# MooreThreads/LiteGS

Hardware: NVIDIA H100
Metric: forward+backward views/sec @1080p 1M Gaussians (higher is better)
Workload: dtype f32

## Files before the change

### include/litegs_b200.h

```cpp
#ifndef LITEGS_B200_H
#define LITEGS_B200_H

#include <stddef.h>
#include <stdint.h>

#ifdef __cplusplus
extern "C" {
#endif

#define LGS_ERR_ARG 10001
#define LGS_ERR_WORKSPACE 10002
#define LGS_REC_FLOATS 12
#define LGS_GRAD_FLOATS 12

const char* lgs_last_error(void);
int lgs_abi_version(void);


int lgs_frustum_culling_aabb(const float* aabb_origin, const float* aabb_ext, const float* frustumplane, int M, int V,
                             uint8_t* visibility, int* visible_num, int64_t* visible_chunk_id, void* stream);

int lgs_cull_compact_activate(int sh_degree, const int64_t* visible_chunk_id, const int* visible_chunks_num,
                              const float* view_matrix, int V, const float* position, const float* scale,
                              const float* rotation, const float* sh_base, const float* sh_rest, const float* opacity,
                              int C, int S, int A, float* act_position, float* act_scale, float* act_rotation,
                              float* color, float* act_opacity, void* stream);

int lgs_activate_backward(int sh_degree, const int64_t* visible_chunk_id, const int* visible_chunks_num,
                          const float* view_matrix, int V, const float* position, const float* scale,
                          const float* rotation, const float* opacity, int C, int S, int A, int rest_dim,
                          int true_sigmoid_grad, const float* g_act_position, const float* g_act_scale,
                          const float* g_act_rotation, const float* g_color, const float* g_act_opacity,
                          float* g_position, float* g_scale, float* g_rotation, float* g_sh_base, float* g_sh_rest,
                          float* g_opacity, void* stream);


int lgs_mvp_transform_forward(const float* world_position, const float* view_matrix, const float* proj_matrix,
                              const int* valid_length, int V, int N, float* view_position, float* ndc_position, void* stream);
int lgs_mvp_transform_backward(const float* grad_ndc_pos, const float* grad_view_pos, const float* view_matrix,
                               const float* proj_matrix, const float* view_pos, const int* valid_length, int V, int N,
                               float* grad_world_pos, void* stream);

int lgs_create_transform_matrix_forward(const float* quaternion, const float* scale, const int* valid_length, int N,
                                        float* transform, void* stream);
int lgs_create_transform_matrix_backward(const float* transform_grad, const float* quaternion, const float* scale,
                                         const int* valid_length, int N, float* grad_quaternion, float* grad_scale,
                                         void* stream);

int lgs_jacobian_rayspace(const float* view_pos, const float* proj_matrix, const int* valid_length, int V, int N,
                          int output_h, int output_w, float* jacobian, void* stream);

int lgs_create_cov2d_forward(const float* J, const float* view_matrix, const float* transform_matrix,
                             const int* valid_length, int V, int N, float* cov2d, void* stream);
int lgs_create_cov2d_backward(const float* cov2d_grad, const float* J, const float* view_matrix,
                              const float* transform_matrix, const int* valid_length, int V, int N,
                              float* transform_matrix_grad, void* stream);

int lgs_eigh_and_inv_2x2_forward(const float* input, const int* valid_length, int V, int N, float* val, float* vec,
                                 float* inv, void* stream);
int lgs_inv_2x2_backward(const float* inv_matrix, const float* grad_inv, const int* valid_length, int V, int N,
                         float* grad_matrix, void* stream);

int lgs_sh2rgb_forward(int degree, const float* sh_base, const float* sh_rest, const float* dirs, int V, int N,
                       float* rgb, void* stream);
int lgs_sh2rgb_backward(int degree, const float* rgb_grad, int sh_rest_dim, const float* dirs, int V, int N,
                        float* sh_base_grad, float* sh_rest_grad, float* dir_grad, void* stream);


int lgs_get_allocate_size(const float* ndc, const float* view_space_z, const float* inv_cov2d, const float* opacity,
                          const int* valid_length, int V, int N, int height, int width, int tile_h, int tile_w,
                          int* left_up, int* right_down, int* allocate_size, void* stream);

int lgs_create_table_workspace_bytes(int V, int cap, size_t* bytes);
int lgs_create_table(const float* ndc, const float* inv_cov2d, const float* opacity, const int* offset,
                     const int64_t* depth_sorted_pointid, int V, int N, int cap, int height, int width, int tile_h,
                     int tile_w, int* sorted_tile_id, int* sorted_point_id, void* workspace, size_t workspace_bytes,
                     void* stream);

int lgs_tile_range(const int* table_tile_id, int V, int table_length, int max_tile_id, int fix_last, int* tile_range,
                   void* stream);

int lgs_tile_range_u16(const unsigned short* table_tile_id, int V, int table_length, int max_tile_id, int fix_last,
                       int* tile_range, void* stream);

int lgs_set_sort_impl(int impl);
int lgs_set_radix_form(int onesweep);
int lgs_sort_pairs_u16_workspace_bytes(int n, size_t* bytes);
int lgs_sort_pairs_u16(const unsigned short* keys_in, unsigned short* keys_out, const unsigned* vals_in, unsigned* vals_out,
                       int n, int begin_bit, int end_bit, void* workspace, size_t workspace_bytes, void* stream);
int lgs_sort_pairs_u32_workspace_bytes(int n, size_t* bytes);
int lgs_sort_pairs_u32(const unsigned* keys_in, unsigned* keys_out, const unsigned* vals_in, unsigned* vals_out, int n,
                       int begin_bit, int end_bit, void* workspace, size_t workspace_bytes, void* stream);
int lgs_sort_pairs_u32_rebased(const unsigned* keys_in, unsigned* keys_out, const unsigned* vals_in, unsigned* vals_out, int n,
                               unsigned bias, int end_bit, void* workspace, size_t workspace_bytes, void* stream);
int lgs_scan_gathered_workspace_bytes(int n, size_t* bytes);
int lgs_scan_gathered(const int* counts, const unsigned* order, int n, int* out, void* workspace,
                      size_t workspace_bytes, void* stream);

int lgs_view_params(const int* counters , int S, int pair_capacity,
                    int planned_depth_bits, int* params ,
                    int* sticky , void* stream);
int lgs_sort_pairs_u32_dev(const unsigned* keys_in, unsigned* keys_out, const unsigned* vals_in, unsigned* vals_out, int capacity,
                           const int* n_dev, const unsigned* bias_dev, int end_bit, void* workspace, size_t workspace_bytes, void* stream);
int lgs_sort_pairs_u16_dev(const unsigned short* keys_in, unsigned short* keys_out, const unsigned* vals_in, unsigned* vals_out,
                           int capacity, const int* n_dev, int begin_bit, int end_bit, void* workspace, size_t workspace_bytes,
                           void* stream);
int lgs_sort_pairs_u32k_dev(const unsigned* keys_in, unsigned* keys_out, const unsigned* vals_in, unsigned* vals_out, int capacity,
                            const int* n_dev, int begin_bit, int end_bit, void* workspace, size_t workspace_bytes, void* stream);
int lgs_scan_gathered_dev(const int* counts, const unsigned* order, int capacity, const int* n_dev, int* out, void* workspace,
                          size_t workspace_bytes, void* stream);
int lgs_emit_pairs_dev(const float* packed_params, const int* offset, const unsigned* order, int n_capacity, const int* n_dev, int cap,
                       int img_h, int img_w, int tile_h, int tile_w, int key_bits , void* keys, int* vals,
                       int* valid_pairs , void* stream);
int lgs_tile_range_u16_dev(const unsigned short* table_tile_id, int capacity, const int* length_dev, int max_tile_id, int fix_last,
                           int* tile_range, void* stream);
int lgs_tile_range_dev(const int* table_tile_id, int capacity, const int* length_dev, int max_tile_id, int fix_last, int* tile_range,
                       void* stream);


int lgs_pack_params(const float* ndc, const float* cov2d_inv, const float* color, const float* opacity, int V, int N,
                    int img_h, int img_w, float* packed_params, void* stream);

int lgs_rasterize_forward_packed(const int* sorted_points, const int* start_index, const float* packed_params,
                                 const int* specific_tiles, int n_specific, int V, int N, int cap, int img_h, int img_w,
                                 int tile_h, int tile_w, int enable_statistic, int clamp_zero, float* img,
                                 float* transmittance, short* last_contributor, int* fragment_count,
                                 float* fragment_weight, int* tile_work, void* stream);

int lgs_tile_order(const int* work, int V, int ntile, int* order, void* stream);

int lgs_rasterize_backward(const int* sorted_points, const int* start_index, const float* packed_params,
                           const int* specific_tiles, int n_specific, const float* final_transmittance,
                           const short* last_contributor, const float* d_img, const float* d_trans_img,
                           const float* clamped_img, const float* grad_inv_scaler, int V, int N, int cap, int img_h, int img_w, int tile_h,
                           int tile_w, int enable_statistic, float* packed_grad, float* d_ndc, float* d_cov2d_inv,
                           float* d_color, float* d_opacity, float* err_sum, float* err_square_sum, void* stream);

int lgs_set_staging(int bulk);
int lgs_set_backward_reduce(int deferred);
int lgs_set_warps_per_block(int wpb);
int lgs_set_forward_pairs(int on);
int lgs_set_backward_kernel(int version);
int lgs_set_deterministic(int on);
int lgs_set_err_square_mode(int mode);


int lgs_project_forward(int sh_degree, const int64_t* visible_chunk_id, const int* visible_chunks_num,
                        const float* view_matrix, const float* proj_matrix, const float* position, const float* scale,
                        const float* rotation, const float* sh_base, const float* sh_rest, const float* opacity, int C,
                        int S, int A, int img_h, int img_w, int tile_h, int tile_w, float* packed_params,
                        unsigned* depth_key, unsigned* iota, int* tile_count, int* totals, const float* filter_3d, int antialiased,
                        void* stream);

int lgs_emit_pairs(const float* packed_params, const int* offset, const unsigned* order, int n, int cap, int img_h,
                   int img_w, int tile_h, int tile_w, int* keys, int* vals, void* stream);
int lgs_emit_pairs_u16(const float* packed_params, const int* offset, const unsigned* order, int n, int cap, int img_h,
                       int img_w, int tile_h, int tile_w, unsigned short* keys, int* vals, void* stream);

int lgs_project_backward(int sh_degree, const int64_t* visible_chunk_id, const int* visible_chunks_num,
                         const float* view_matrix, const float* proj_matrix, const float* position, const float* scale,
                         const float* rotation, const float* opacity, int C, int S, int A, int rest_dim, int img_h,
                         int img_w, int true_sigmoid_grad, const float* packed_grad, const float* grad_inv_scaler,
                         int zero_outputs, float* g_position, float* g_scale, float* g_rotation, float* g_sh_base,
                         float* g_sh_rest, float* g_opacity, float* touched, float* cam_partials, float* d_cam,
                         const float* filter_3d, int antialiased, void* stream);

int lgs_create_viewproj_forward(const float* view_params, const float* recp_tan_half_fov_x, int V, int img_h, int img_w,
                                float z_near, float z_far, float* view_matrix, float* proj_matrix, float* viewproj_matrix,
                                float* frustumplane, void* stream);
int lgs_create_viewproj_backward(const float* view_matrix_grad, const float* proj_matrix_grad, const float* viewproj_matrix_grad,
                                 const float* view_params, const float* recp_tan_half_fov_x, int V, int img_h, int img_w,
                                 float z_near, float z_far, float* grad_view_params, float* grad_recp_tan_half_fov_x, void* stream);


int lgs_adam_update_chunk(float* param, const float* grad, float* exp_avg, float* exp_avg_sq,
                          const int64_t* visible_index, const int* valid_length, int R, int C, int S, int A, double lr,
                          double b1, double b2, double eps, void* stream);
int lgs_adam_update_primitive(float* param, const float* grad, float* exp_avg, float* exp_avg_sq,
                              const int64_t* primitive_visible, int R, int N, double lr, double b1, double b2,
                              double eps, void* stream);

int lgs_mark_visible_chunks(const int64_t* visible_chunk_id, const int* visible_chunks_num, int A, float* touched, void* stream);
int lgs_adam_step_dense(float* const* params, const int* rows_per_param, const float* lr_per_param, float* grad,
                        float* exp_avg, float* exp_avg_sq, float* touched, int C, int S, double b1, double b2, double eps,
                        int clear_grad, void* stream);

int lgs_sparse_chunk_op(void* A, const void* B, const int64_t* visible_chunk_ids, const int* visible_count, int dtype,
                        int op, int ele_num, int chunks, int alloc_chunks, int chunk_size, void* stream);

int lgs_nvls_allreduce_f32(float* multicast_ptr, size_t n_floats, int rank, int world, int ctas, void* stream);


int lgs_morton_codes(const float* xyz, const float* lo3, const float* hi3, int N, int bits, long long* codes, void* stream);
int lgs_permute_rows(const float* src, const long long* idx, int R, int N, float* dst, void* stream);
int lgs_cluster_aabb(const float* xyz, const float* scale, const float* rot, int C, int S, float* origin, float* extend, void* stream);
int lgs_filter_3d(const float* position, int C, int S, const float* view, const float* proj, const int* hw, int V,
                  float* filter_3d, void* stream);


int lgs_ssim_num_block_sums(int B, int CH, int H, int W, int* count);
int lgs_ssim_forward(const float* img1, const float* img2, int B, int CH, int H, int W, float C1, float C2, int l1_mode,
                     float ssim_weight, float* map, float* dm_dmu1, float* dm_dsigma1_sq, float* dm_dsigma12,
                     float* block_sums, void* stream);
int lgs_ssim_backward(const float* img1, const float* img2, const float* dL_dmap, float uniform_chain, const float* dm_dmu1,
                      const float* dm_dsigma1_sq, const float* dm_dsigma12, int B, int CH, int H, int W, int l1_mode,
                      float ssim_weight, float* dL_dimg1, void* stream);

#ifdef __cplusplus
}
#endif
#endif
```

### litegs_b200/_lib.py

```python
from __future__ import annotations

import ctypes
import os

_HERE = os.path.dirname(os.path.abspath(__file__))
LIB_PATH = os.environ.get("LITEGS_B200_LIB") or os.path.join(_HERE, "liblitegs_b200.so")

_P, _I, _D, _Z, _F = ctypes.c_void_p, ctypes.c_int, ctypes.c_double, ctypes.c_size_t, ctypes.c_float

SIGNATURES = {
    "lgs_frustum_culling_aabb": [_P, _P, _P, _I, _I, _P, _P, _P, _P],
    "lgs_cull_compact_activate": [_I, _P, _P, _P, _I, _P, _P, _P, _P, _P, _P, _I, _I, _I, _P, _P, _P, _P, _P, _P],
    "lgs_activate_backward": [_I, _P, _P, _P, _I, _P, _P, _P, _P, _I, _I, _I, _I, _I, _P, _P, _P, _P, _P,
                              _P, _P, _P, _P, _P, _P, _P],
    "lgs_mvp_transform_forward": [_P, _P, _P, _P, _I, _I, _P, _P, _P],
    "lgs_mvp_transform_backward": [_P, _P, _P, _P, _P, _P, _I, _I, _P, _P],
    "lgs_create_transform_matrix_forward": [_P, _P, _P, _I, _P, _P],
    "lgs_create_transform_matrix_backward": [_P, _P, _P, _P, _I, _P, _P, _P],
    "lgs_jacobian_rayspace": [_P, _P, _P, _I, _I, _I, _I, _P, _P],
    "lgs_create_cov2d_forward": [_P, _P, _P, _P, _I, _I, _P, _P],
    "lgs_create_cov2d_backward": [_P, _P, _P, _P, _P, _I, _I, _P, _P],
    "lgs_eigh_and_inv_2x2_forward": [_P, _P, _I, _I, _P, _P, _P, _P],
    "lgs_inv_2x2_backward": [_P, _P, _P, _I, _I, _P, _P],
    "lgs_sh2rgb_forward": [_I, _P, _P, _P, _I, _I, _P, _P],
    "lgs_sh2rgb_backward": [_I, _P, _I, _P, _I, _I, _P, _P, _P, _P],
    "lgs_get_allocate_size": [_P, _P, _P, _P, _P, _I, _I, _I, _I, _I, _I, _P, _P, _P, _P],
    "lgs_create_table_workspace_bytes": [_I, _I, ctypes.POINTER(_Z)],
    "lgs_create_table": [_P, _P, _P, _P, _P, _I, _I, _I, _I, _I, _I, _I, _P, _P, _P, _Z, _P],
    "lgs_tile_range": [_P, _I, _I, _I, _I, _P, _P],
    "lgs_tile_range_u16": [_P, _I, _I, _I, _I, _P, _P],
    "lgs_sort_pairs_u16_workspace_bytes": [_I, ctypes.POINTER(_Z)],
    "lgs_sort_pairs_u16": [_P, _P, _P, _P, _I, _I, _I, _P, _Z, _P],
    "lgs_emit_pairs_u16": [_P, _P, _P, _I, _I, _I, _I, _I, _I, _P, _P, _P],
    "lgs_sort_pairs_u32_workspace_bytes": [_I, ctypes.POINTER(_Z)],
    "lgs_sort_pairs_u32": [_P, _P, _P, _P, _I, _I, _I, _P, _Z, _P],
    "lgs_sort_pairs_u32_rebased": [_P, _P, _P, _P, _I, ctypes.c_uint, _I, _P, _Z, _P],
    "lgs_scan_gathered_workspace_bytes": [_I, ctypes.POINTER(_Z)],
    "lgs_scan_gathered": [_P, _P, _I, _P, _P, _Z, _P],
    "lgs_view_params": [_P, _I, _I, _I, _P, _P, _P],
    "lgs_sort_pairs_u32_dev": [_P, _P, _P, _P, _I, _P, _P, _I, _P, _Z, _P],
    "lgs_sort_pairs_u16_dev": [_P, _P, _P, _P, _I, _P, _I, _I, _P, _Z, _P],
    "lgs_sort_pairs_u32k_dev": [_P, _P, _P, _P, _I, _P, _I, _I, _P, _Z, _P],
    "lgs_scan_gathered_dev": [_P, _P, _I, _P, _P, _P, _Z, _P],
    "lgs_emit_pairs_dev": [_P, _P, _P, _I, _P, _I, _I, _I, _I, _I, _I, _P, _P, _P, _P],
    "lgs_tile_range_u16_dev": [_P, _I, _P, _I, _I, _P, _P],
    "lgs_tile_range_dev": [_P, _I, _P, _I, _I, _P, _P],
    "lgs_pack_params": [_P, _P, _P, _P, _I, _I, _I, _I, _P, _P],
    "lgs_rasterize_forward_packed": [_P, _P, _P, _P, _I, _I, _I, _I, _I, _I, _I, _I, _I, _I, _P, _P, _P, _P, _P, _P, _P],
    "lgs_tile_order": [_P, _I, _I, _P, _P],
    "lgs_rasterize_backward": [_P, _P, _P, _P, _I, _P, _P, _P, _P, _P, _P, _I, _I, _I, _I, _I, _I, _I, _I,
                               _P, _P, _P, _P, _P, _P, _P, _P],
    "lgs_set_staging": [_I],
    "lgs_set_sort_impl": [_I],
    "lgs_set_radix_form": [_I],
    "lgs_set_warps_per_block": [_I],
    "lgs_set_backward_reduce": [_I],
    "lgs_set_backward_kernel": [_I],
    "lgs_set_forward_pairs": [_I],
    "lgs_set_err_square_mode": [_I],
    "lgs_set_deterministic": [_I],
    "lgs_project_forward": [_I, _P, _P, _P, _P, _P, _P, _P, _P, _P, _P, _I, _I, _I, _I, _I, _I, _I, _P, _P, _P, _P, _P, _P, _I, _P],
    "lgs_emit_pairs": [_P, _P, _P, _I, _I, _I, _I, _I, _I, _P, _P, _P],
    "lgs_project_backward": [_I, _P, _P, _P, _P, _P, _P, _P, _P, _I, _I, _I, _I, _I, _I, _I, _P, _P, _I,
                             _P, _P, _P, _P, _P, _P, _P, _P, _P, _P, _I, _P],
    "lgs_create_viewproj_forward": [_P, _P, _I, _I, _I, _F, _F, _P, _P, _P, _P, _P],
    "lgs_create_viewproj_backward": [_P, _P, _P, _P, _P, _I, _I, _I, _F, _F, _P, _P, _P],
    "lgs_adam_update_chunk": [_P, _P, _P, _P, _P, _P, _I, _I, _I, _I, _D, _D, _D, _D, _P],
    "lgs_adam_update_primitive": [_P, _P, _P, _P, _P, _I, _I, _D, _D, _D, _D, _P],
    "lgs_sparse_chunk_op": [_P, _P, _P, _P, _I, _I, _I, _I, _I, _I, _P],
    "lgs_mark_visible_chunks": [_P, _P, _I, _P, _P],
    "lgs_nvls_allreduce_f32": [_P, _Z, _I, _I, _I, _P],
    "lgs_morton_codes": [_P, _P, _P, _I, _I, _P, _P],
    "lgs_permute_rows": [_P, _P, _I, _I, _P, _P],
    "lgs_cluster_aabb": [_P, _P, _P, _I, _I, _P, _P, _P],
    "lgs_filter_3d": [_P, _I, _I, _P, _P, _P, _I, _P, _P],
    "lgs_adam_step_dense": [_P, _P, _P, _P, _P, _P, _P, _I, _I, _D, _D, _D, _I, _P],
    "lgs_ssim_num_block_sums": [_I, _I, _I, _I, ctypes.POINTER(_I)],
    "lgs_ssim_forward": [_P, _P, _I, _I, _I, _I, _F, _F, _I, _F, _P, _P, _P, _P, _P, _P],
    "lgs_ssim_backward": [_P, _P, _P, _F, _P, _P, _P, _I, _I, _I, _I, _I, _F, _P, _P],
}
NO_STATUS = {"lgs_last_error": ctypes.c_char_p, "lgs_abi_version": ctypes.c_int}

_lib = None


class LiteGSB200Error(RuntimeError):
    pass


def load() -> ctypes.CDLL:
    global _lib
    if _lib is not None:
        return _lib
    if not os.path.exists(LIB_PATH):
        raise LiteGSB200Error(
            f"{LIB_PATH} not found: build it with `python -m litegs_b200.build` (nvcc, sm_90a). "
            "litegs_b200 has no CPU or PyTorch fallback.")
    lib = ctypes.CDLL(LIB_PATH)
    for name, argtypes in SIGNATURES.items():
        fn = getattr(lib, name)
        fn.argtypes = argtypes
        fn.restype = ctypes.c_int
    for name, restype in NO_STATUS.items():
        fn = getattr(lib, name)
        fn.argtypes = []
        fn.restype = restype
    _lib = lib
    return lib


def exported_symbols():
    return list(SIGNATURES) + list(NO_STATUS)


def call(name: str, *args) -> None:
    lib = load()
    rc = getattr(lib, name)(*args)
    if rc != 0:
        msg = lib.lgs_last_error()
        raise LiteGSB200Error(f"{name} failed (code {rc}): {msg.decode() if msg else ''}")
```

### litegs_b200/csrc/raster.cu

```cuda
#include "common.cuh"

#define FULL_MASK 0xffffffffu
#define LOG2E 1.4426950408889634f
#define ALPHA_MIN (1.0f / 256.0f)
#define ALPHA_MAX (255.0f / 256.0f)
#define T_MIN (1.0f / 8192.0f)
#define WARPS_PER_BLOCK 4

__device__ __forceinline__ float fast_ex2(float x)
{
    float y;
    asm("ex2.approx.ftz.f32 %0, %1;" : "=f"(y) : "f"(x));
    return y;
}
__device__ __forceinline__ float fast_rcp(float x)
{
    float y;
    asm("rcp.approx.ftz.f32 %0, %1;" : "=f"(y) : "f"(x));
    return y;
}

__device__ __forceinline__ float2 add2(float2 a, float2 b) { return make_float2(__fadd_rn(a.x, b.x), __fadd_rn(a.y, b.y)); }
__device__ __forceinline__ float2 mul2(float2 a, float2 b) { return make_float2(__fmul_rn(a.x, b.x), __fmul_rn(a.y, b.y)); }
__device__ __forceinline__ float2 fma2(float2 a, float2 b, float2 c) { return make_float2(__fmaf_rn(a.x, b.x, c.x), __fmaf_rn(a.y, b.y, c.y)); }

__device__ __forceinline__ void blend_pixel(float a, float cr, float cg, float cb, float& Ts, float& Cr, float& Cg, float& Cb,
                                            float& nf, float ts_min, float a_min, float neg_ki)
{
    asm("{\n"
        ".reg .pred pa, pk;\n"
        ".reg .f32 w;\n"
        "setp.gt.f32 pa, %0, %9;\n"
        "@pa add.f32 %4, %4, 0f3F800000;\n"
        "setp.ge.and.f32 pk, %5, %10, pa;\n"
        "mul.f32 w, %5, %0;\n"
        "@pk fma.rn.f32 %1, %6, w, %1;\n"
        "@pk fma.rn.f32 %2, %7, w, %2;\n"
        "@pk fma.rn.f32 %3, %8, w, %3;\n"
        "@pk fma.rn.f32 %0, %11, w, %0;\n"
        "}\n"
        : "+f"(Ts), "+f"(Cr), "+f"(Cg), "+f"(Cb), "+f"(nf)
        : "f"(a), "f"(cr), "f"(cg), "f"(cb), "f"(ts_min), "f"(a_min), "f"(neg_ki));
}

__device__ __forceinline__ unsigned smem_u32(const void* p) { return (unsigned)__cvta_generic_to_shared(p); }
__device__ __forceinline__ void cp_async16(void* dst, const void* src)
{
    asm volatile("cp.async.cg.shared.global [%0], [%1], 16;\n" ::"r"(smem_u32(dst)), "l"(src));
}
__device__ __forceinline__ void cp_async_commit() { asm volatile("cp.async.commit_group;\n" ::); }
template <int N> __device__ __forceinline__ void cp_async_wait() { asm volatile("cp.async.wait_group %0;\n" ::"n"(N)); }

__device__ __forceinline__ void mbar_init(uint64_t* bar, unsigned count)
{
    asm volatile("mbarrier.init.shared::cta.b64 [%0], %1;\n" ::"r"(smem_u32(bar)), "r"(count));
}
__device__ __forceinline__ void mbar_expect_tx(uint64_t* bar, unsigned bytes)
{
    asm volatile("mbarrier.arrive.expect_tx.shared::cta.b64 _, [%0], %1;\n" ::"r"(smem_u32(bar)), "r"(bytes));
}
__device__ __forceinline__ bool mbar_try_wait(uint64_t* bar, unsigned parity)
{
    unsigned ok;
    asm volatile(
        "{\n"
        ".reg .pred p;\n"
        "mbarrier.try_wait.parity.shared::cta.b64 p, [%1], %2;\n"
        "selp.u32 %0, 1, 0, p;\n"
        "}\n"
        : "=r"(ok)
        : "r"(smem_u32(bar)), "r"(parity)
        : "memory");
    return ok != 0;
}
__device__ __forceinline__ void mbar_wait(uint64_t* bar, unsigned parity)
{
    while (!mbar_try_wait(bar, parity)) {}
}
__device__ __forceinline__ void bulk_g2s(void* dst, const void* src, unsigned bytes, uint64_t* bar)
{
    asm volatile("cp.async.bulk.shared::cluster.global.mbarrier::complete_tx::bytes [%0], [%1], %2, [%3];\n" ::"r"(smem_u32(dst)),
                 "l"(src), "r"(bytes), "r"(smem_u32(bar))
                 : "memory");
}

template <bool BULK>
struct Stager {
    SplatRec* buf;
    uint64_t* bar;
    unsigned phase_bits;
    unsigned pending;
    int lane;
    __device__ __forceinline__ void init(SplatRec* b, uint64_t* m, int ln)
    {
        buf = b; bar = m; lane = ln; phase_bits = 0; pending = 0;
        if (BULK) {
            if (lane == 0) { mbar_init(&bar[0], 1); mbar_init(&bar[1], 1); }
            asm volatile("fence.mbarrier_init.release.cluster;\n" ::);
            __syncwarp();
        }
    }
    __device__ __forceinline__ void issue(int which, const SplatRec* __restrict__ recs, int id)
    {
        SplatRec* dst = buf + which * 32 + lane;
        if (BULK) {
            unsigned live = __ballot_sync(FULL_MASK, id >= 0);
            if (lane == 0) mbar_expect_tx(&bar[which], (unsigned)__popc(live) * (unsigned)sizeof(SplatRec));
            __syncwarp();
            if (id >= 0) bulk_g2s(dst, recs + id, (unsigned)sizeof(SplatRec), &bar[which]);
            pending |= (1u << which);
        } else {
            if (id >= 0) {
                const char* src = (const char*)(recs + id);
                cp_async16((char*)dst, src);
                cp_async16((char*)dst + 16, src + 16);
                cp_async16((char*)dst + 32, src + 32);
            }
            cp_async_commit();
        }
    }
    template <bool PRE = false>
    __device__ __forceinline__ void wait(int which, bool more_in_flight)
    {
        if (BULK) {
            mbar_wait(&bar[which], (phase_bits >> which) & 1u);
            phase_bits ^= (1u << which);
            pending &= ~(1u << which);
            if (PRE) { prescale(which); __syncwarp(); }
        } else {
            if (more_in_flight) cp_async_wait<1>(); else cp_async_wait<0>();
            if (PRE) prescale(which);
            __syncwarp();
        }
    }
    __device__ __forceinline__ void prescale(int which)
    {
        SplatRec* r = buf + which * 32 + lane;
        const float2 ab = *reinterpret_cast<const float2*>(&r->A);
        const float2 co = *reinterpret_cast<const float2*>(&r->C);
        *reinterpret_cast<float2*>(&r->A) = make_float2((-0.5f * LOG2E) * ab.x, (-LOG2E) * ab.y);
        r->C = (-0.5f * LOG2E) * co.x;
        r->depth = co.y * (256.0f / 255.0f);
    }
    __device__ __forceinline__ void drain()
    {
        if (BULK) {
            if (pending & 1u) wait(0, false);
            if (pending & 2u) wait(1, false);
        } else {
            cp_async_wait<0>();
        }
    }
};

__global__ void pack_kernel(const float* __restrict__ ndc, const float* __restrict__ inv_cov, const float* __restrict__ color,
                            const float* __restrict__ opac, SplatRec* __restrict__ recs, int N, int H, int W)
{
    int i = blockIdx.x * blockDim.x + threadIdx.x, b = blockIdx.y;
    if (i >= N) return;
    size_t o4 = (size_t)b * 4 * N + i, o3 = (size_t)b * 3 * N + i;
    SplatRec r;
    r.px = __fsub_rn(__fmul_rn(__fmul_rn(__fadd_rn(ndc[o4], 1.0f), 0.5f), (float)W), 0.5f);
    r.py = __fsub_rn(__fmul_rn(__fmul_rn(__fadd_rn(ndc[o4 + N], 1.0f), 0.5f), (float)H), 0.5f);
    r.depth = ndc[o4 + 2 * (size_t)N];
    r.A = inv_cov[o4]; r.B = inv_cov[o4 + N]; r.C = inv_cov[o4 + 3 * (size_t)N];
    r.o = opac[i];
    r.r = color[o3]; r.g = color[o3 + N]; r.b = color[o3 + 2 * (size_t)N];
    r.pad0 = 0.f; r.pad1 = 0.f;
    recs[(size_t)b * N + i] = r;
}

template <int TH, int TW, bool STAT, bool BULK, bool PAIRS = false>
__global__ void __launch_bounds__(32 * WARPS_PER_BLOCK) raster_forward_kernel(
    const int* __restrict__ sorted, const int* __restrict__ start_index, const SplatRec* __restrict__ recs,
    const int* __restrict__ tiles, int n_sel, float* __restrict__ img, float* __restrict__ Tout, unsigned short* __restrict__ last,
    int* __restrict__ frag_count, float* __restrict__ frag_weight, int* __restrict__ tile_work, int gx, int ntile, int cap, int N,
    int Hp, int Wp, int clamp_zero)
{
    constexpr int PPT = TH * TW / 32;
    __shared__ __align__(128) SplatRec s_rec[WARPS_PER_BLOCK][2][32];
    __shared__ __align__(8) uint64_t s_bar[WARPS_PER_BLOCK][2];
    const int lane = threadIdx.x, warp = threadIdx.y, b = blockIdx.y;
    const int slot = blockIdx.x * blockDim.y + warp;
    int tile_id;
    if (tiles != nullptr) tile_id = (slot < n_sel) ? tiles[(size_t)b * n_sel + slot] : 0;
    else tile_id = slot + 1;
    if (tile_id <= 0 || tile_id > ntile) return;

    const int* rg = start_index + (size_t)b * (ntile + 2);
    const int start = rg[tile_id];
    int count = (start < 0) ? 0 : (rg[tile_id + 1] - start);
    if (count < 0) count = 0;
    recs += (size_t)b * N;
    const int* ids = sorted + (size_t)b * cap + (start < 0 ? 0 : start);

    const int x = ((tile_id - 1) % gx) * TW + lane % TW;
    const int y0 = ((tile_id - 1) / gx) * TH + (lane / TW) * PPT;
    const float fx = (float)x, fy0 = (float)y0;

    constexpr float KS = 256.0f / 255.0f, KI = 255.0f / 256.0f;
    constexpr float TS_MIN = T_MIN * KI, A_MIN_S = ALPHA_MIN * KS;
    float Ts[PPT], Cr[PPT], Cg[PPT], Cb[PPT], nf[PPT];
#pragma unroll
    for (int j = 0; j < PPT; j++) { Ts[j] = KI; Cr[j] = Cg[j] = Cb[j] = 0.0f; nf[j] = 0.0f; }

    if (count > 0) {
        Stager<BULK> st;
        st.init(&s_rec[warp][0][0], &s_bar[warp][0], lane);
        const int nchunks = (count + 31) >> 5;
        int id_cur = (lane < count) ? ids[lane] : -1;
        st.issue(0, recs, id_cur);
        int id_next = (32 + lane < count) ? ids[32 + lane] : -1;
        bool done = false;
        for (int c = 0; c < nchunks && !done; c++) {
            const bool more = (c + 1 < nchunks);
            if (more) {
                st.issue((c + 1) & 1, recs, id_next);
                int nn = (c + 2) * 32 + lane;
                id_next = (nn < count) ? ids[nn] : -1;
            }
            st.template wait<true>(c & 1, more);
            const SplatRec* chunk = &s_rec[warp][c & 1][0];
            const int nk = min(32, count - c * 32);
            int my_id = 0;
            if (STAT) my_id = ids[c * 32 + min(lane, nk - 1)];
            for (int k = 0; k < nk; k++) {
                if ((k & 3) == 0) {
                    float tmax = Ts[0];
#pragma unroll
                    for (int j = 1; j < PPT; j++) tmax = fmaxf(tmax, Ts[j]);
                    if (!__any_sync(FULL_MASK, tmax > TS_MIN)) { done = true; break; }
                }
                const float4 q0 = *reinterpret_cast<const float4*>(&chunk[k].px);
                const float4 q1 = *reinterpret_cast<const float4*>(&chunk[k].C);
                const float2 q2 = *reinterpret_cast<const float2*>(&chunk[k].b);
                const float cb = q2.x;
                const float dx = q0.x - fx, dy0 = q0.y - fy0;
                const float a2 = q0.z, b2 = q0.w, c2 = q1.x;
                const float base = a2 * dx * dx, lin = b2 * dx;
                const float os = q2.y;
                int fcount = 0; float wsum = 0.f;
                if (PAIRS && !STAT) {
                    const float2 dy02 = make_float2(dy0, dy0), c22 = make_float2(c2, c2), lin2 = make_float2(lin, lin),
                                 base2 = make_float2(base, base), os2 = make_float2(os, os);
                    const float2 cr2 = make_float2(q1.z, q1.z), cg2 = make_float2(q1.w, q1.w), cb2 = make_float2(cb, cb),
                                 nki2 = make_float2(-KI, -KI);
#pragma unroll
                    for (int p = 0; p < PPT / 2; p++) {
                        const float2 dy = add2(dy02, make_float2(-(float)(2 * p), -(float)(2 * p + 1)));
                        const float2 pw = fma2(dy, fma2(c22, dy, lin2), base2);
                        const float2 t = mul2(os2, make_float2(fast_ex2(pw.x), fast_ex2(pw.y)));
                        const float a0 = __saturatef(t.x), a1 = __saturatef(t.y);
                        const bool act0 = Ts[2 * p] > TS_MIN, act1 = Ts[2 * p + 1] > TS_MIN;
                        if (act0) nf[2 * p] += 1.0f;
                        if (act1) nf[2 * p + 1] += 1.0f;
                        const float2 aw = make_float2((act0 && a0 >= A_MIN_S) ? a0 : 0.0f, (act1 && a1 >= A_MIN_S) ? a1 : 0.0f);
                        const float2 w = mul2(aw, make_float2(Ts[2 * p], Ts[2 * p + 1]));
                        const float2 r2 = fma2(cr2, w, make_float2(Cr[2 * p], Cr[2 * p + 1]));
                        const float2 g2 = fma2(cg2, w, make_float2(Cg[2 * p], Cg[2 * p + 1]));
                        const float2 b2_ = fma2(cb2, w, make_float2(Cb[2 * p], Cb[2 * p + 1]));
                        const float2 tn = fma2(nki2, w, make_float2(Ts[2 * p], Ts[2 * p + 1]));
                        Cr[2 * p] = r2.x; Cr[2 * p + 1] = r2.y; Cg[2 * p] = g2.x; Cg[2 * p + 1] = g2.y;
                        Cb[2 * p] = b2_.x; Cb[2 * p + 1] = b2_.y; Ts[2 * p] = tn.x; Ts[2 * p + 1] = tn.y;
                    }
                } else {
#pragma unroll
                for (int j = 0; j < PPT; j++) {
                    const float dy = dy0 - (float)j;
                    const float pw = fmaf(dy, fmaf(c2, dy, lin), base);
                    const float a = __saturatef(os * fast_ex2(pw));
                    if (STAT) {
                        const bool ok = (Ts[j] > TS_MIN) && (a >= A_MIN_S);
                        if (ok) { fcount++; wsum += a * Ts[j]; }
                    }
                    blend_pixel(a, q1.z, q1.w, cb, Ts[j], Cr[j], Cg[j], Cb[j], nf[j], TS_MIN, A_MIN_S, -KI);
                }
                }
                if (STAT) {
                    fcount = __reduce_add_sync(FULL_MASK, fcount);
#pragma unroll
                    for (int o = 16; o > 0; o >>= 1) wsum += __shfl_xor_sync(FULL_MASK, wsum, o);
                    int pid = __shfl_sync(FULL_MASK, my_id, k);
                    if (lane == 0 && fcount > 0) {
                        atomicAdd(&frag_count[(size_t)b * N + pid], fcount);
                        atomicAdd(&frag_weight[(size_t)b * N + pid], wsum);
                    }
                }
            }
            __syncwarp();
        }
        st.drain();
    }

    const size_t plane = (size_t)Hp * Wp;
#pragma unroll
    for (int j = 0; j < PPT; j++) {
        const size_t po = (size_t)(y0 + j) * Wp + x;
        const float lo = clamp_zero ? 0.0f : -3.4028234663852886e38f;
        img[((size_t)b * 3 + 0) * plane + po] = fmaxf(fminf(Cr[j], 1.0f), lo);
        img[((size_t)b * 3 + 1) * plane + po] = fmaxf(fminf(Cg[j], 1.0f), lo);
        img[((size_t)b * 3 + 2) * plane + po] = fmaxf(fminf(Cb[j], 1.0f), lo);
        Tout[(size_t)b * plane + po] = Ts[j] * KS;
        last[(size_t)b * plane + po] = (unsigned short)__float2uint_rn(fminf(nf[j], 65535.0f));
    }
    if (tile_work != nullptr) {
        float m = nf[0];
#pragma unroll
        for (int j = 1; j < PPT; j++) m = fmaxf(m, nf[j]);
        const int mi = __reduce_max_sync(FULL_MASK, (int)fminf(m, 65535.0f));
        if (lane == 0) tile_work[(size_t)b * ntile + tile_id - 1] = mi;
    }
}

__device__ __forceinline__ float butterfly8(const float (&v)[8], int lane)
{
    const bool h16 = lane & 16, h8 = lane & 8, h4 = lane & 4;
    float u[4], w[2];
#pragma unroll
    for (int i = 0; i < 4; i++) {
        float send = h16 ? v[i] : v[i + 4], keep = h16 ? v[i + 4] : v[i];
        u[i] = keep + __shfl_xor_sync(FULL_MASK, send, 16);
    }
#pragma unroll
    for (int i = 0; i < 2; i++) {
        float send = h8 ? u[i] : u[i + 2], keep = h8 ? u[i + 2] : u[i];
        w[i] = keep + __shfl_xor_sync(FULL_MASK, send, 8);
    }
    float send = h4 ? w[0] : w[1], keep = h4 ? w[1] : w[0];
    float z = keep + __shfl_xor_sync(FULL_MASK, send, 4);
    z += __shfl_xor_sync(FULL_MASK, z, 2);
    z += __shfl_xor_sync(FULL_MASK, z, 1);
    return z;
}

#define LGS_RG 3
#define LGS_ROWF 36
template <int TH, int TW, bool STAT, bool TRANS, bool BULK, bool DEFER>
__global__ void __launch_bounds__(32 * WARPS_PER_BLOCK) raster_backward_kernel(
    const int* __restrict__ sorted, const int* __restrict__ start_index, const SplatRec* __restrict__ recs,
    const int* __restrict__ tiles, int n_sel, const float* __restrict__ Tfinal, const unsigned short* __restrict__ last,
    const float* __restrict__ d_img, const float* __restrict__ d_trans, const float* __restrict__ clamped_img,
    float* __restrict__ grad, int gx, int ntile, int cap, int N, int Hp, int Wp)
{
    constexpr int PPT = TH * TW / 32;
    constexpr int NV = STAT ? 10 : 9;
    constexpr float KS = 256.0f / 255.0f, A_MIN_S = ALPHA_MIN * KS;
    __shared__ __align__(128) SplatRec s_rec[WARPS_PER_BLOCK][2][32];
    __shared__ __align__(8) uint64_t s_bar[WARPS_PER_BLOCK][2];
    __shared__ __align__(16) float s_acc[DEFER ? WARPS_PER_BLOCK : 1][DEFER ? LGS_RG * NV : 1][LGS_ROWF];
    const int lane = threadIdx.x, warp = threadIdx.y, b = blockIdx.y;
    const int slot = blockIdx.x * blockDim.y + warp;
    int tile_id;
    if (tiles != nullptr) tile_id = (slot < n_sel) ? tiles[(size_t)b * n_sel + slot] : 0;
    else tile_id = slot + 1;
    if (tile_id <= 0 || tile_id > ntile) return;
    const int* rg = start_index + (size_t)b * (ntile + 2);
    const int start = rg[tile_id];
    if (start < 0) return;
    recs += (size_t)b * N;
    grad += (size_t)b * N * LGS_GRAD_FLOATS;
    const int* ids = sorted + (size_t)b * cap + start;

    const int x = ((tile_id - 1) % gx) * TW + lane % TW;
    const int y0 = ((tile_id - 1) / gx) * TH + (lane / TW) * PPT;
    const float fx = (float)x, fy0 = (float)y0;
    const size_t plane = (size_t)Hp * Wp;

    float T[PPT], g0[PPT], g1[PPT], g2[PPT], S[PPT], gt[PPT];
    int nl[PPT];
    int kmax = 0;
#pragma unroll
    for (int j = 0; j < PPT; j++) {
        const size_t po = (size_t)(y0 + j) * Wp + x;
        T[j] = Tfinal[(size_t)b * plane + po];
        g0[j] = d_img[((size_t)b * 3 + 0) * plane + po];
        g1[j] = d_img[((size_t)b * 3 + 1) * plane + po];
        g2[j] = d_img[((size_t)b * 3 + 2) * plane + po];
        if (clamped_img != nullptr) {
            if (!(clamped_img[((size_t)b * 3 + 0) * plane + po] > 0.0f)) g0[j] = 0.0f;
            if (!(clamped_img[((size_t)b * 3 + 1) * plane + po] > 0.0f)) g1[j] = 0.0f;
            if (!(clamped_img[((size_t)b * 3 + 2) * plane + po] > 0.0f)) g2[j] = 0.0f;
        }
        gt[j] = TRANS ? d_trans[(size_t)b * plane + po] * T[j] : 0.0f;
        S[j] = 0.0f;
        nl[j] = (int)last[(size_t)b * plane + po];
        kmax = max(kmax, nl[j]);
    }
    kmax = __reduce_max_sync(FULL_MASK, kmax);
    if (kmax <= 0) return;

    int pend = 0, pid0 = 0, pid1 = 0, pid2 = 0;
    auto flush = [&]() {
        __syncwarp();
        if (lane < pend * NV) {
            const float4* r4 = reinterpret_cast<const float4*>(&s_acc[DEFER ? warp : 0][DEFER ? lane : 0][0]);
            float4 x0 = r4[0], x1 = r4[1], x2 = r4[2], x3 = r4[3], x4 = r4[4], x5 = r4[5], x6 = r4[6], x7 = r4[7];
            float sum = (((x0.x + x0.y) + (x0.z + x0.w)) + ((x1.x + x1.y) + (x1.z + x1.w))) +
                        (((x2.x + x2.y) + (x2.z + x2.w)) + ((x3.x + x3.y) + (x3.z + x3.w))) +
                        ((((x4.x + x4.y) + (x4.z + x4.w)) + ((x5.x + x5.y) + (x5.z + x5.w))) +
                         (((x6.x + x6.y) + (x6.z + x6.w)) + ((x7.x + x7.y) + (x7.z + x7.w))));
            const int sp = lane / NV, v = lane - sp * NV;
            const int pid = sp == 0 ? pid0 : (sp == 1 ? pid1 : pid2);
            atomicAdd(&grad[(size_t)pid * LGS_GRAD_FLOATS + v], sum);
        }
        __syncwarp();
        pend = 0;
    };
    Stager<BULK> st;
    st.init(&s_rec[warp][0][0], &s_bar[warp][0], lane);
    const int nchunks = (kmax + 31) >> 5;
    int c0 = nchunks - 1;
    int id_cur = (c0 * 32 + lane < kmax) ? ids[c0 * 32 + lane] : -1;
    st.issue(0, recs, id_cur);
    int id_next = (c0 >= 1) ? ids[(c0 - 1) * 32 + lane] : -1;
    for (int v = 0; v < nchunks; v++) {
        const int c = nchunks - 1 - v;
        const bool more = (c >= 1);
        const int id_this = id_cur;
        if (more) {
            st.issue((v + 1) & 1, recs, id_next);
            id_cur = id_next;
            id_next = (c >= 2) ? ids[(c - 2) * 32 + lane] : -1;
        }
        st.wait(v & 1, more);
        const SplatRec* chunk = &s_rec[warp][v & 1][0];
        const int nk = min(32, kmax - c * 32);
        for (int kk = nk - 1; kk >= 0; kk--) {
            const int k = c * 32 + kk;
            const float4 q0 = *reinterpret_cast<const float4*>(&chunk[kk].px);
            const float4 q1 = *reinterpret_cast<const float4*>(&chunk[kk].C);
            const float cb = chunk[kk].b;
            const float dx = q0.x - fx, dy0 = q0.y - fy0;
            const float a2 = (-0.5f * LOG2E) * q0.z, b2 = (-LOG2E) * q0.w, c2 = (-0.5f * LOG2E) * q1.x;
            const float base = a2 * dx * dx, lin = b2 * dx;
            const float os = q1.y * KS;
            float s0 = 0.f, s1 = 0.f, s2 = 0.f, dr = 0.f, dg = 0.f, db = 0.f, esq = 0.f;
            bool any = false;
#pragma unroll
            for (int j = 0; j < PPT; j++) {
                const float dy = dy0 - (float)j;
                const float pw = fmaf(dy, fmaf(c2, dy, lin), base);
                const float G = fast_ex2(pw);
                const float at = q1.y * G;
                if (k < nl[j] && os * G >= A_MIN_S) {
                    any = true;
                    const float a = fminf(at, ALPHA_MAX);
                    const float rc = fast_rcp(1.0f - a);
                    const float Tj = fminf(1.0f, T[j] * rc);
                    T[j] = Tj;
                    const float w = a * Tj;
                    dr = fmaf(w, g0[j], dr); dg = fmaf(w, g1[j], dg); db = fmaf(w, g2[j], db);
                    const float diff = fmaf(q1.z, g0[j], fmaf(q1.w, g1[j], cb * g2[j])) - S[j];
                    float da = Tj * diff;
                    if (TRANS) da -= gt[j] * rc;
                    S[j] = fmaf(a, diff, S[j]);
                    if (STAT) { const float go = G * da; esq = fmaf(go, go, esq); }
                    const float dpw = at * da;
                    s0 += dpw; s1 = fmaf(dpw, dy, s1); s2 = fmaf(dpw * dy, dy, s2);
                }
            }
            if (__any_sync(FULL_MASK, any)) {
                float v8[8];
                const float u0 = dx * s0;
                v8[0] = u0;
                v8[1] = s1;
                v8[2] = dx * u0;
                v8[3] = dx * s1;
                v8[4] = s2;
                v8[5] = dr; v8[6] = dg; v8[7] = db;
                float dop = s0;
                const int pid = __shfl_sync(FULL_MASK, id_this, kk);
                if (DEFER) {
                    float* row = &s_acc[DEFER ? warp : 0][DEFER ? pend * NV : 0][lane];
#pragma unroll
                    for (int v = 0; v < 8; v++) row[v * LGS_ROWF] = v8[v];
                    row[8 * LGS_ROWF] = dop;
                    if (STAT) row[9 * LGS_ROWF] = esq;
                    if (pend == 0) pid0 = pid; else if (pend == 1) pid1 = pid; else pid2 = pid;
                    pend++;
                    if (pend == LGS_RG) flush();
                } else {
                    const float tot = butterfly8(v8, lane);
#pragma unroll
                    for (int o = 16; o > 0; o >>= 1) dop += __shfl_xor_sync(FULL_MASK, dop, o);
                    if (STAT) {
#pragma unroll
                        for (int o = 16; o > 0; o >>= 1) esq += __shfl_xor_sync(FULL_MASK, esq, o);
                    }
                    int slotv = -1; float val = 0.f;
                    if ((lane & 3) == 0) { slotv = ((lane >> 4) & 1) * 4 + ((lane >> 3) & 1) * 2 + ((lane >> 2) & 1); val = tot; }
                    else if (lane == 1) { slotv = 8; val = dop; }
                    else if (STAT && lane == 2) { slotv = 9; val = esq; }
                    if (slotv >= 0) atomicAdd(&grad[(size_t)pid * LGS_GRAD_FLOATS + slotv], val);
                }
            }
        }
        __syncwarp();
    }
    if (DEFER && pend > 0) flush();
    st.drain();
}

__device__ __forceinline__ float2 bc2(float a) { return make_float2(a, a); }

#define LGS_DET_SCALE 68719476736.0
template <int TH, int TW, bool STAT, bool TRANS, bool DET = false>
__global__ void __launch_bounds__(32 * WARPS_PER_BLOCK) raster_backward_v2_kernel(
    const int* __restrict__ sorted, const int* __restrict__ start_index, const SplatRec* __restrict__ recs,
    const int* __restrict__ tiles, int n_sel, const float* __restrict__ Tfinal, const unsigned short* __restrict__ last,
    const float* __restrict__ d_img, const float* __restrict__ d_trans, const float* __restrict__ clamped_img,
    float* __restrict__ grad, int gx, int ntile, int cap, int N, int Hp, int Wp, int err_mode)
{
    constexpr int PPT = TH * TW / 32, NP = PPT / 2;
    static_assert(PPT % 2 == 0, "pixels per lane must pair up");
    constexpr int NV = STAT ? 10 : 9;
    constexpr float KS = 256.0f / 255.0f, A_MIN_S = ALPHA_MIN * KS;
    __shared__ __align__(128) SplatRec s_rec[WARPS_PER_BLOCK][2][32];
    __shared__ __align__(8) uint64_t s_bar[WARPS_PER_BLOCK][2];
    __shared__ __align__(16) float s_acc[WARPS_PER_BLOCK][LGS_RG * NV][LGS_ROWF];
    __shared__ int s_pid[WARPS_PER_BLOCK][4];
    const int lane = threadIdx.x, warp = threadIdx.y, b = blockIdx.y;
    const int slot = blockIdx.x * blockDim.y + warp;
    int tile_id;
    if (tiles != nullptr) tile_id = (slot < n_sel) ? tiles[(size_t)b * n_sel + slot] : 0;
    else tile_id = slot + 1;
    if (tile_id <= 0 || tile_id > ntile) return;
    const int* rg = start_index + (size_t)b * (ntile + 2);
    const int start = rg[tile_id];
    if (start < 0) return;
    recs += (size_t)b * N;
    grad += (size_t)b * N * LGS_GRAD_FLOATS * (DET ? 2 : 1);
    const int* ids = sorted + (size_t)b * cap + start;

    const int x = ((tile_id - 1) % gx) * TW + lane % TW;
    const int y0 = ((tile_id - 1) / gx) * TH + (lane / TW) * PPT;
    const float fx = (float)x, fy0 = (float)y0;
    const size_t plane = (size_t)Hp * Wp;

    float2 T[NP], g0[NP], g1[NP], g2[NP], S[NP], ngt[NP];
    int nl[PPT];
    int kmax = 0;
#pragma unroll
    for (int j = 0; j < PPT; j++) {
        const size_t po = (size_t)(y0 + j) * Wp + x;
        float t = Tfinal[(size_t)b * plane + po];
        float a0 = d_img[((size_t)b * 3 + 0) * plane + po];
        float a1 = d_img[((size_t)b * 3 + 1) * plane + po];
        float a2 = d_img[((size_t)b * 3 + 2) * plane + po];
        if (clamped_img != nullptr) {
            if (!(clamped_img[((size_t)b * 3 + 0) * plane + po] > 0.0f)) a0 = 0.0f;
            if (!(clamped_img[((size_t)b * 3 + 1) * plane + po] > 0.0f)) a1 = 0.0f;
            if (!(clamped_img[((size_t)b * 3 + 2) * plane + po] > 0.0f)) a2 = 0.0f;
        }
        const float gtj = TRANS ? -(d_trans[(size_t)b * plane + po] * t) : 0.0f;
        if (j & 1) { T[j / 2].y = t; g0[j / 2].y = a0; g1[j / 2].y = a1; g2[j / 2].y = a2; ngt[j / 2].y = gtj; S[j / 2].y = 0.f; }
        else       { T[j / 2].x = t; g0[j / 2].x = a0; g1[j / 2].x = a1; g2[j / 2].x = a2; ngt[j / 2].x = gtj; S[j / 2].x = 0.f; }
        nl[j] = (int)last[(size_t)b * plane + po];
        kmax = max(kmax, nl[j]);
    }
    kmax = __reduce_max_sync(FULL_MASK, kmax);
    if (kmax <= 0) return;

    int pend = 0;
    auto flush = [&]() {
        __syncwarp();
        if (lane < pend * NV) {
            const float4* r4 = reinterpret_cast<const float4*>(&s_acc[warp][lane][0]);
            const float4 x0 = r4[0], x1 = r4[1], x2 = r4[2], x3 = r4[3], x4 = r4[4], x5 = r4[5], x6 = r4[6], x7 = r4[7];
            float2 p0 = add2(make_float2(x0.x, x0.y), make_float2(x0.z, x0.w));
            float2 p1 = add2(make_float2(x1.x, x1.y), make_float2(x1.z, x1.w));
            float2 p2 = add2(make_float2(x2.x, x2.y), make_float2(x2.z, x2.w));
            float2 p3 = add2(make_float2(x3.x, x3.y), make_float2(x3.z, x3.w));
            float2 p4 = add2(make_float2(x4.x, x4.y), make_float2(x4.z, x4.w));
            float2 p5 = add2(make_float2(x5.x, x5.y), make_float2(x5.z, x5.w));
            float2 p6 = add2(make_float2(x6.x, x6.y), make_float2(x6.z, x6.w));
            float2 p7 = add2(make_float2(x7.x, x7.y), make_float2(x7.z, x7.w));
            p0 = add2(p0, p1); p2 = add2(p2, p3); p4 = add2(p4, p5); p6 = add2(p6, p7);
            p0 = add2(p0, p2); p4 = add2(p4, p6);
            p0 = add2(p0, p4);
            const float sum = p0.x + p0.y;
            const int sp = lane / NV, v = lane - sp * NV;
            const int pid = s_pid[warp][sp];
            if (DET) {
                unsigned long long* gq = reinterpret_cast<unsigned long long*>(grad);
                atomicAdd(&gq[(size_t)pid * LGS_GRAD_FLOATS + v], (unsigned long long)__double2ll_rn((double)sum * LGS_DET_SCALE));
            } else {
                atomicAdd(&grad[(size_t)pid * LGS_GRAD_FLOATS + v], sum);
            }
        }
        __syncwarp();
        pend = 0;
    };
    Stager<false> st;
    st.init(&s_rec[warp][0][0], &s_bar[warp][0], lane);
    const int nchunks = (kmax + 31) >> 5;
    int c0 = nchunks - 1;
    int id_cur = (c0 * 32 + lane < kmax) ? ids[c0 * 32 + lane] : -1;
    st.issue(0, recs, id_cur);
    int id_next = (c0 >= 1) ? ids[(c0 - 1) * 32 + lane] : -1;
    for (int v = 0; v < nchunks; v++) {
        const int c = nchunks - 1 - v;
        const bool more = (c >= 1);
        const int id_this = id_cur;
        if (more) {
            st.issue((v + 1) & 1, recs, id_next);
            id_cur = id_next;
            id_next = (c >= 2) ? ids[(c - 2) * 32 + lane] : -1;
        }
        st.template wait<true>(v & 1, more);
        const SplatRec* chunk = &s_rec[warp][v & 1][0];
        const int nk = min(32, kmax - c * 32);
        for (int kk = nk - 1; kk >= 0; kk--) {
            const int k = c * 32 + kk;
            const float4 q0 = *reinterpret_cast<const float4*>(&chunk[kk].px);
            const float4 q1 = *reinterpret_cast<const float4*>(&chunk[kk].C);
            const float2 q2 = *reinterpret_cast<const float2*>(&chunk[kk].b);
            const float cb = q2.x;
            const float dx = q0.x - fx, dy0 = q0.y - fy0;
            const float a2 = q0.z, b2 = q0.w, c2 = q1.x;
            const float base = a2 * dx * dx, lin = b2 * dx;
            const float2 os2 = bc2(q2.y), o2 = bc2(q1.y), c22 = bc2(c2), lin2 = bc2(lin), base2 = bc2(base);
            const float2 cr2 = bc2(q1.z), cg2 = bc2(q1.w), cb2 = bc2(cb), dy02 = bc2(dy0);
            float2 s0, s1, s2, dr, dg, db;
            float esq = 0.f, runx = 0.f, runy = 0.f;
            bool any = false;
#pragma unroll
            for (int p = 0; p < NP; p++) {
                const float2 dy = add2(dy02, make_float2(-(float)(2 * p), -(float)(2 * p + 1)));
                const float2 pw = fma2(dy, fma2(c22, dy, lin2), base2);
                float2 G = make_float2(fast_ex2(pw.x), fast_ex2(pw.y));
                const float2 tt = mul2(os2, G);
                const bool ok0 = (tt.x >= A_MIN_S) && (k < nl[2 * p]);
                const bool ok1 = (tt.y >= A_MIN_S) && (k < nl[2 * p + 1]);
                any |= ok0 | ok1;
                G.x = ok0 ? G.x : 0.0f;
                G.y = ok1 ? G.y : 0.0f;
                const float2 at = mul2(o2, G);
                const float2 a = make_float2(fminf(at.x, ALPHA_MAX), fminf(at.y, ALPHA_MAX));
                const float2 om = fma2(a, bc2(-1.0f), bc2(1.0f));
                const float2 rc = make_float2(fast_rcp(om.x), fast_rcp(om.y));
                const float2 Tn = mul2(T[p], rc);
                T[p] = Tn;
                const float2 w = mul2(a, Tn);
                const float2 cgd = fma2(cr2, g0[p], fma2(cg2, g1[p], mul2(cb2, g2[p])));
                const float2 diff = fma2(S[p], bc2(-1.0f), cgd);
                float2 da = mul2(Tn, diff);
                if (TRANS) da = fma2(ngt[p], rc, da);
                S[p] = fma2(a, diff, S[p]);
                const float2 dpw = mul2(at, da);
                const float2 td = mul2(dpw, dy);
                if (p == 0) {
                    dr = mul2(w, g0[p]); dg = mul2(w, g1[p]); db = mul2(w, g2[p]);
                    s0 = dpw; s1 = td; s2 = mul2(td, dy);
                } else {
                    dr = fma2(w, g0[p], dr); dg = fma2(w, g1[p], dg); db = fma2(w, g2[p], db);
                    s0 = add2(s0, dpw);
                    s1 = add2(s1, td);
                    s2 = fma2(td, dy, s2);
                }
                if (STAT) {
                    const float2 go = mul2(G, da);
                    if (err_mode == 1) {
                        if (__any_sync(FULL_MASK, ok0 | ok1)) {
                            runx += go.x; runy += go.y;
                            esq = fmaf(runx, runx, fmaf(runy, runy, esq));
                        }
                    } else {
                        esq = fmaf(go.x, go.x, fmaf(go.y, go.y, esq));
                    }
                }
            }
            if (__any_sync(FULL_MASK, any)) {
                const float m0 = s0.x + s0.y, m1 = s1.x + s1.y, m2 = s2.x + s2.y;
                const float u0 = dx * m0;
                if (lane == kk) s_pid[warp][pend] = id_this;
                float* row = &s_acc[warp][pend * NV][lane];
                row[0 * LGS_ROWF] = u0;
                row[1 * LGS_ROWF] = m1;
                row[2 * LGS_ROWF] = dx * u0;
                row[3 * LGS_ROWF] = dx * m1;
                row[4 * LGS_ROWF] = m2;
                row[5 * LGS_ROWF] = dr.x + dr.y;
                row[6 * LGS_ROWF] = dg.x + dg.y;
                row[7 * LGS_ROWF] = db.x + db.y;
                row[8 * LGS_ROWF] = m0;
                if (STAT) row[9 * LGS_ROWF] = esq;
                pend++;
                if (pend == LGS_RG) flush();
            }
        }
        __syncwarp();
    }
    if (pend > 0) flush();
    st.drain();
}

__global__ void det_to_float_kernel(const long long* __restrict__ q, float* __restrict__ g, size_t n)
{
    size_t i = (size_t)blockIdx.x * blockDim.x + threadIdx.x;
    if (i < n) g[i] = (float)((double)q[i] * (1.0 / LGS_DET_SCALE));
}

__global__ void unpack_kernel(const float* __restrict__ grad, const SplatRec* __restrict__ recs, const float* __restrict__ inv_scaler,
                              int N, int H, int W, float* __restrict__ d_ndc, float* __restrict__ d_cov, float* __restrict__ d_color,
                              float* __restrict__ d_opac, float* __restrict__ err_sum, float* __restrict__ err_sq)
{
    int i = blockIdx.x * blockDim.x + threadIdx.x, b = blockIdx.y;
    if (i >= N) return;
    const float s = inv_scaler ? inv_scaler[0] : 1.0f;
    const float4* g4 = reinterpret_cast<const float4*>(grad + ((size_t)b * N + i) * LGS_GRAD_FLOATS);
    const float4 a = g4[0], c = g4[1], e = g4[2];
    const SplatRec r = recs[(size_t)b * N + i];
    LgsRasterGrad g;
    lgs_finish_raster_grad(a, c, e, r.A, r.B, r.C, r.o, g);
    size_t o4 = (size_t)b * 4 * N + i, o3 = (size_t)b * 3 * N + i;
    d_ndc[o4] = g.dmx * 0.5f * W * s; d_ndc[o4 + N] = g.dmy * 0.5f * H * s;
    d_ndc[o4 + 2 * (size_t)N] = 0.f; d_ndc[o4 + 3 * (size_t)N] = 0.f;
    d_cov[o4] = g.dA * s; d_cov[o4 + N] = g.dB * 0.5f * s; d_cov[o4 + 2 * (size_t)N] = g.dB * 0.5f * s; d_cov[o4 + 3 * (size_t)N] = g.dC * s;
    d_color[o3] = c.y * s; d_color[o3 + N] = c.z * s; d_color[o3 + 2 * (size_t)N] = c.w * s;
    if (b == 0) d_opac[i] = g.dop * s;
    if (err_sum) err_sum[(size_t)b * N + i] = 0.f;
    if (err_sq) err_sq[(size_t)b * N + i] = e.y;
}

__global__ void __launch_bounds__(1024) tile_order_kernel(const int* __restrict__ work, int ntile, int* __restrict__ order)
{
    __shared__ int s_cnt[1024];
    __shared__ int s_warp[32];
    const int t = threadIdx.x, b = blockIdx.x;
    const int* w = work + (size_t)b * ntile;
    s_cnt[t] = 0;
    __syncthreads();
    for (int i = t; i < ntile; i += 1024) atomicAdd(&s_cnt[1023 - min(max(w[i], 0) >> 2, 1023)], 1);
    __syncthreads();
    const int c = s_cnt[t];
    int incl = c;
#pragma unroll
    for (int o = 1; o < 32; o <<= 1) { int v = __shfl_up_sync(FULL_MASK, incl, o); if ((t & 31) >= o) incl += v; }
    if ((t & 31) == 31) s_warp[t >> 5] = incl;
    __syncthreads();
    if (t < 32) {
        int v = s_warp[t], in2 = v;
#pragma unroll
        for (int o = 1; o < 32; o <<= 1) { int u = __shfl_up_sync(FULL_MASK, in2, o); if (t >= o) in2 += u; }
        s_warp[t] = in2 - v;
    }
    __syncthreads();
    s_cnt[t] = incl - c + s_warp[t >> 5];
    __syncthreads();
    for (int i = t; i < ntile; i += 1024) {
        const int pos = atomicAdd(&s_cnt[1023 - min(max(w[i], 0) >> 2, 1023)], 1);
        order[(size_t)b * ntile + pos] = i + 1;
    }
}

extern "C" int lgs_tile_order(const int* work, int V, int ntile, int* order, void* stream)
{
    LGS_REQUIRE(V >= 1 && ntile >= 1, "tile_order: bad sizes V=%d tiles=%d", V, ntile);
    tile_order_kernel<<<V, 1024, 0, (cudaStream_t)stream>>>(work, ntile, order);
    LGS_CHECK_LAUNCH("tile_order_kernel");
    return LGS_OK;
}

static int g_use_bulk = -1;
static bool use_bulk()
{
    if (g_use_bulk < 0) {
        const char* e = getenv("LGS_STAGING");
        g_use_bulk = (e && e[0] == 'b') ? 1 : 0;
    }
    return g_use_bulk == 1;
}
extern "C" int lgs_set_staging(int bulk) { g_use_bulk = bulk ? 1 : 0; return LGS_OK; }

static int g_defer = -1;
static bool use_deferred_reduce()
{
    if (g_defer < 0) {
        const char* e = getenv("LGS_BWD_REDUCE");
        g_defer = (e && e[0] == 'b') ? 0 : 1;
    }
    return g_defer == 1;
}
extern "C" int lgs_set_backward_reduce(int deferred) { g_defer = deferred ? 1 : 0; return LGS_OK; }

static int g_fwd_pairs = -1;
static bool forward_pairs()
{
    if (g_fwd_pairs < 0) {
        const char* e = getenv("LGS_FWD_PAIRS");
        g_fwd_pairs = (e && e[0] == '1') ? 1 : 0;
    }
    return g_fwd_pairs == 1;
}
extern "C" int lgs_set_forward_pairs(int on) { g_fwd_pairs = on ? 1 : 0; return LGS_OK; }

static int g_bwd = -1;
static int backward_version()
{
    if (g_bwd < 0) {
        const char* e = getenv("LGS_BWD");
        g_bwd = (e && (e[0] == '1' || (e[0] == 'v' && e[1] == '1'))) ? 1 : 2;
    }
    return g_bwd;
}
extern "C" int lgs_set_backward_kernel(int version)
{
    LGS_REQUIRE(version == 1 || version == 2, "set_backward_kernel: %d not in {1,2}", version);
    g_bwd = version;
    return LGS_OK;
}

static int g_err_mode = 1;
extern "C" int lgs_set_err_square_mode(int mode)
{
    LGS_REQUIRE(mode == 0 || mode == 1, "set_err_square_mode: %d not in {0,1}", mode);
    g_err_mode = mode;
    return LGS_OK;
}

static int g_det = -1;
static bool deterministic()
{
    if (g_det < 0) {
        const char* e = getenv("LGS_DETERMINISTIC");
        g_det = (e && e[0] == '1') ? 1 : 0;
    }
    return g_det == 1;
}
extern "C" int lgs_set_deterministic(int on) { g_det = on ? 1 : 0; return LGS_OK; }

static int g_wpb = -1;
static int warps_per_block()
{
    if (g_wpb < 0) {
        const char* e = getenv("LGS_WPB");
        int v = e ? atoi(e) : 4;
        g_wpb = (v == 1 || v == 2 || v == 4) ? v : 4;
    }
    return g_wpb;
}
extern "C" int lgs_set_warps_per_block(int wpb)
{
    LGS_REQUIRE(wpb == 1 || wpb == 2 || wpb == 4, "set_warps_per_block: %d not in {1,2,4}", wpb);
    g_wpb = wpb;
    return LGS_OK;
}

extern "C" int lgs_pack_params(const float* ndc, const float* cov2d_inv, const float* color, const float* opacity, int V, int N,
                               int img_h, int img_w, float* packed_params, void* stream)
{
    if (N == 0) return LGS_OK;
    pack_kernel<<<dim3(lgs_cdiv(N, 256), V), 256, 0, (cudaStream_t)stream>>>(ndc, cov2d_inv, color, opacity, (SplatRec*)packed_params, N,
                                                                           img_h, img_w);
    LGS_CHECK_LAUNCH("pack_kernel");
    return LGS_OK;
}

extern "C" int lgs_rasterize_forward_packed(const int* sorted_points, const int* start_index, const float* packed_params,
                                            const int* specific_tiles, int n_specific, int V, int N, int cap, int img_h, int img_w,
                                            int tile_h, int tile_w, int enable_statistic, int clamp_zero, float* img,
                                            float* transmittance, short* last_contributor, int* fragment_count,
                                            float* fragment_weight, int* tile_work, void* stream)
{
    LGS_REQUIRE(lgs_tile_ok(tile_h, tile_w), "rasterize_forward: tile %dx%d not one of 8x16, 12x16, 16x16, 8x8", tile_h, tile_w);
    LGS_REQUIRE(V >= 1 && img_h > 0 && img_w > 0, "rasterize_forward: bad sizes V=%d H=%d W=%d", V, img_h, img_w);
    int gx = (img_w + tile_w - 1) / tile_w, gy = (img_h + tile_h - 1) / tile_h;
    int ntile = gx * gy, Hp = gy * tile_h, Wp = gx * tile_w;
    int nrender = specific_tiles ? n_specific : ntile;
    if (nrender == 0) return LGS_OK;
    const int wpb = warps_per_block();
    dim3 grid(lgs_cdiv(nrender, wpb), V), block(32, wpb);
    cudaStream_t st = (cudaStream_t)stream;
    const SplatRec* recs = (const SplatRec*)packed_params;
    const bool bulk = use_bulk();
#define FWD(S, B) raster_forward_kernel<TH, TW, S, B><<<grid, block, 0, st>>>(sorted_points, start_index, recs, specific_tiles, n_specific, \
        img, transmittance, (unsigned short*)last_contributor, fragment_count, fragment_weight, tile_work, gx, ntile, cap, N, Hp, Wp, clamp_zero)
#define FWDP() raster_forward_kernel<TH, TW, false, false, true><<<grid, block, 0, st>>>(sorted_points, start_index, recs, specific_tiles, \
        n_specific, img, transmittance, (unsigned short*)last_contributor, fragment_count, fragment_weight, tile_work, gx, ntile, cap, N, Hp, Wp, clamp_zero)
    LGS_DISPATCH_TILE(tile_h, tile_w,
        if (enable_statistic) { if (bulk) FWD(true, true); else FWD(true, false); }
        else { if (bulk) FWD(false, true); else if (forward_pairs()) FWDP(); else FWD(false, false); })
#undef FWD
#undef FWDP
    LGS_CHECK_LAUNCH("raster_forward_kernel");
    return LGS_OK;
}

extern "C" int lgs_rasterize_backward(const int* sorted_points, const int* start_index, const float* packed_params,
                                      const int* specific_tiles, int n_specific, const float* final_transmittance,
                                      const short* last_contributor, const float* d_img, const float* d_trans_img,
                                      const float* clamped_img, const float* grad_inv_scaler, int V, int N, int cap, int img_h,
                                      int img_w, int tile_h,
                                      int tile_w, int enable_statistic, float* packed_grad, float* d_ndc, float* d_cov2d_inv,
                                      float* d_color, float* d_opacity, float* err_sum, float* err_square_sum, void* stream)
{
    LGS_REQUIRE(lgs_tile_ok(tile_h, tile_w), "rasterize_backward: tile %dx%d not one of 8x16, 12x16, 16x16, 8x8", tile_h, tile_w);
    LGS_REQUIRE(V >= 1 && img_h > 0 && img_w > 0, "rasterize_backward: bad sizes V=%d H=%d W=%d", V, img_h, img_w);
    int gx = (img_w + tile_w - 1) / tile_w, gy = (img_h + tile_h - 1) / tile_h;
    int ntile = gx * gy, Hp = gy * tile_h, Wp = gx * tile_w;
    int nrender = specific_tiles ? n_specific : ntile;
    cudaStream_t st = (cudaStream_t)stream;
    if (N == 0) return LGS_OK;
    LGS_CUDA(cudaMemsetAsync(packed_grad, 0, sizeof(float) * (size_t)V * N * LGS_GRAD_FLOATS, st));
    if (nrender > 0) {
        const int wpb = warps_per_block();
        dim3 grid(lgs_cdiv(nrender, wpb), V), block(32, wpb);
        const SplatRec* recs = (const SplatRec*)packed_params;
        const bool bulk = use_bulk();
        const bool trans = d_trans_img != nullptr;
        const bool defer = use_deferred_reduce() && !bulk;
        const unsigned short* lastu = (const unsigned short*)last_contributor;
        if (deterministic()) {
            const size_t nq = (size_t)V * N * LGS_GRAD_FLOATS;
            long long* q = nullptr;
            LGS_CUDA(cudaMallocAsync((void**)&q, nq * sizeof(long long), st));
            LGS_CUDA(cudaMemsetAsync(q, 0, nq * sizeof(long long), st));
#define BWD_DET(S, T) raster_backward_v2_kernel<TH, TW, S, T, true><<<grid, block, 0, st>>>(sorted_points, start_index, recs, specific_tiles, \
        n_specific, final_transmittance, lastu, d_img, d_trans_img, clamped_img, (float*)q, gx, ntile, cap, N, Hp, Wp, g_err_mode)
            LGS_DISPATCH_TILE(tile_h, tile_w,
                if (enable_statistic) { if (trans) BWD_DET(true, true); else BWD_DET(true, false); }
                else { if (trans) BWD_DET(false, true); else BWD_DET(false, false); })
#undef BWD_DET
            LGS_CHECK_LAUNCH("raster_backward_v2_kernel<DET>");
            det_to_float_kernel<<<lgs_cdiv((long long)nq, 256), 256, 0, st>>>(q, packed_grad, nq);
            LGS_CHECK_LAUNCH("det_to_float_kernel");
            LGS_CUDA(cudaFreeAsync(q, st));
        } else if (backward_version() == 2 && !bulk) {
#define BW2(S, T) raster_backward_v2_kernel<TH, TW, S, T><<<grid, block, 0, st>>>(sorted_points, start_index, recs, specific_tiles, n_specific, \
        final_transmittance, lastu, d_img, d_trans_img, clamped_img, packed_grad, gx, ntile, cap, N, Hp, Wp, g_err_mode)
            LGS_DISPATCH_TILE(tile_h, tile_w,
                if (enable_statistic) { if (trans) BW2(true, true); else BW2(true, false); }
                else { if (trans) BW2(false, true); else BW2(false, false); })
#undef BW2
            LGS_CHECK_LAUNCH("raster_backward_v2_kernel");
        } else {
#define BWD(S, T, B) if (defer) BWD2(S, T, false, true); else BWD2(S, T, B, false)
#define BWD2(S, T, B, D) raster_backward_kernel<TH, TW, S, T, B, D><<<grid, block, 0, st>>>(sorted_points, start_index, recs, specific_tiles, \
        n_specific, final_transmittance, lastu, d_img, d_trans_img, clamped_img, packed_grad, gx, ntile, cap, N, Hp, Wp)
        LGS_DISPATCH_TILE(tile_h, tile_w,
            if (enable_statistic) { if (trans) { if (bulk) BWD(true, true, true); else BWD(true, true, false); }
                                    else { if (bulk) BWD(true, false, true); else BWD(true, false, false); } }
            else { if (trans) { if (bulk) BWD(false, true, true); else BWD(false, true, false); }
                   else { if (bulk) BWD(false, false, true); else BWD(false, false, false); } })
#undef BWD
#undef BWD2
        LGS_CHECK_LAUNCH("raster_backward_kernel");
        }
    }
    if (d_ndc != nullptr) {
        unpack_kernel<<<dim3(lgs_cdiv(N, 256), V), 256, 0, st>>>(packed_grad, (const SplatRec*)packed_params, grad_inv_scaler, N, img_h, img_w,
                                                                d_ndc, d_cov2d_inv, d_color, d_opacity, err_sum, err_square_sum);
        LGS_CHECK_LAUNCH("unpack_kernel");
    }
    return LGS_OK;
}
```

### litegs_b200/fused.py

```python
from __future__ import annotations

import ctypes
import math
import os
from typing import Optional

import torch

from . import _lib

_F32, _I32, _I64 = torch.float32, torch.int32, torch.int64

CONFIG = {
    "fix_last_tile": True,
    "true_sigmoid_grad": False,
    "tile_order": os.environ.get("LGS_TILE_ORDER", "1") != "0",
}


def _ptr(t: Optional[torch.Tensor]):
    return None if t is None else t.data_ptr()


def _stream(dev):
    return torch.cuda.current_stream(dev).cuda_stream


class _OnDevice:
    __slots__ = ("ctx",)

    def __init__(self, dev):
        self.ctx = None if torch.cuda.current_device() == (dev.index if dev.index is not None else torch.cuda.current_device()) \
            else torch.cuda.device(dev)

    def __enter__(self):
        if self.ctx is not None:
            self.ctx.__enter__()

    def __exit__(self, *a):
        if self.ctx is not None:
            return self.ctx.__exit__(*a)
        return False


_on = _OnDevice


def _f32c(t: torch.Tensor, name: str) -> torch.Tensor:
    if not t.is_cuda:
        raise RuntimeError(f"{name} must be a CUDA tensor (litegs_b200 has no CPU path)")
    if t.dtype != _F32:
        raise RuntimeError(f"{name}: expected float32, got {t.dtype}")
    return t if t.is_contiguous() else t.contiguous()


def _asc(t: torch.Tensor, dtype, name: str) -> torch.Tensor:
    if not t.is_cuda:
        raise RuntimeError(f"{name} must be a CUDA tensor")
    if t.dtype != dtype:
        raise RuntimeError(f"{name}: expected {dtype}, got {t.dtype}")
    return t if t.is_contiguous() else t.contiguous()


def _vl(valid_length: Optional[torch.Tensor]):
    if valid_length is None:
        return None
    return _asc(valid_length, _I32, "valid_length")


def _tiles(img_h, img_w, th, tw):
    gy = (int(img_h) + th - 1) // th
    gx = (int(img_w) + tw - 1) // tw
    return gx, gy



def frustum_culling_aabb(aabb_origin, aabb_ext, frustumplane, feedback_buffer_arg=None, data_idx_arg=None):
    o = _f32c(aabb_origin, "aabb_origin"); e = _f32c(aabb_ext, "aabb_ext"); f = _f32c(frustumplane, "frustumplane")
    M, V = o.shape[1], f.shape[0]
    dev = o.device
    with torch.cuda.device(dev):
        vis = torch.empty(M, dtype=torch.bool, device=dev)
        num = torch.zeros(1, dtype=_I32, device=dev)
        ids = torch.arange(M, dtype=_I64, device=dev)
        _lib.call("lgs_frustum_culling_aabb", _ptr(o), _ptr(e), _ptr(f), M, V, _ptr(vis), _ptr(num), _ptr(ids), _stream(dev))
        pred = 0
        if feedback_buffer_arg is not None and data_idx_arg is not None:
            for i in range(data_idx_arg.shape[0]):
                idx = int(data_idx_arg[i])
                pred = max(pred, int(feedback_buffer_arg[idx]))
                feedback_buffer_arg[idx:idx + 1].copy_(num, non_blocking=True)
        pred = int(1.2 * pred)
        if pred <= 0:
            pred = int(num.item())
        pred = min(pred, M)
    return [vis, num, ids[:pred]]


def cull_compact_activate(sh_degree, visible_chunk_id, visible_chunks_num, view_matrix,
                          position, scale, rotation, sh_base, sh_rest, opacity):
    ids = _asc(visible_chunk_id, _I64, "visible_chunk_id"); num = _asc(visible_chunks_num, _I32, "visible_chunks_num")
    view = _f32c(view_matrix, "view_matrix")
    pos = _f32c(position, "position"); sc = _f32c(scale, "scale"); rot = _f32c(rotation, "rotation")
    s0 = _f32c(sh_base, "sh_base"); sr = _f32c(sh_rest, "sh_rest"); op = _f32c(opacity, "opacity")
    K = (int(sh_degree) + 1) ** 2
    if sr.shape[0] < K - 1:
        raise RuntimeError(f"sh_rest has {sr.shape[0]} rows, sh_degree {sh_degree} needs {K - 1}")
    C, S = pos.shape[-2:]
    A, V = ids.shape[0], view.shape[0]
    dev = pos.device
    with torch.cuda.device(dev):
        apos = torch.empty((4, A, S), dtype=_F32, device=dev)
        asc = torch.empty((3, A, S), dtype=_F32, device=dev)
        arot = torch.empty((4, A, S), dtype=_F32, device=dev)
        color = torch.empty((V, 3, A, S), dtype=_F32, device=dev)
        aop = torch.empty((1, A, S), dtype=_F32, device=dev)
        _lib.call("lgs_cull_compact_activate", int(sh_degree), _ptr(ids), _ptr(num), _ptr(view), V, _ptr(pos), _ptr(sc),
                  _ptr(rot), _ptr(s0), _ptr(sr), _ptr(op), C, S, A, _ptr(apos), _ptr(asc), _ptr(arot), _ptr(color),
                  _ptr(aop), _stream(dev))
    return [apos, asc, arot, color, aop]


def activate_backward(sh_degree, visible_chunk_id, visible_chunks_num, view_matrix,
                      position, scale, rotation, sh_base, sh_rest, opacity,
                      activated_position_grad, activated_scale_grad, activated_rotation_grad, color_grad,
                      activated_opacity_grad):
    ids = _asc(visible_chunk_id, _I64, "visible_chunk_id"); num = _asc(visible_chunks_num, _I32, "visible_chunks_num")
    view = _f32c(view_matrix, "view_matrix")
    pos = _f32c(position, "position"); sc = _f32c(scale, "scale"); rot = _f32c(rotation, "rotation")
    op = _f32c(opacity, "opacity")
    gp = _f32c(activated_position_grad, "activated_position_grad"); gs = _f32c(activated_scale_grad, "activated_scale_grad")
    gr = _f32c(activated_rotation_grad, "activated_rotation_grad"); gc = _f32c(color_grad, "color_grad")
    go = _f32c(activated_opacity_grad, "activated_opacity_grad")
    C, S = pos.shape[-2:]
    A, V, R = ids.shape[0], view.shape[0], sh_rest.shape[0]
    dev = pos.device
    with torch.cuda.device(dev):
        o_pos = torch.empty((3, A, S), dtype=_F32, device=dev)
        o_sc = torch.empty((3, A, S), dtype=_F32, device=dev)
        o_rot = torch.empty((4, A, S), dtype=_F32, device=dev)
        o_s0 = torch.empty((1, 3, A, S), dtype=_F32, device=dev)
        o_sr = torch.empty((R, 3, A, S), dtype=_F32, device=dev)
        o_op = torch.empty((1, A, S), dtype=_F32, device=dev)
        _lib.call("lgs_activate_backward", int(sh_degree), _ptr(ids), _ptr(num), _ptr(view), V, _ptr(pos), _ptr(sc), _ptr(rot),
                  _ptr(op), C, S, A, R, int(CONFIG["true_sigmoid_grad"]), _ptr(gp), _ptr(gs), _ptr(gr), _ptr(gc), _ptr(go),
                  _ptr(o_pos), _ptr(o_sc), _ptr(o_rot), _ptr(o_s0), _ptr(o_sr), _ptr(o_op), _stream(dev))
    return [o_pos, o_sc, o_rot, o_s0, o_sr, o_op]



def mvp_transform_forward(world_position, view_matrix, proj_matrix, valid_length=None):
    p = _f32c(world_position, "world_position"); vm = _f32c(view_matrix, "view_matrix"); pm = _f32c(proj_matrix, "proj_matrix")
    V, N = vm.shape[0], p.shape[1]
    dev = p.device
    with torch.cuda.device(dev):
        vp = torch.empty((V, 4, N), dtype=_F32, device=dev)
        ndc = torch.empty((V, 4, N), dtype=_F32, device=dev)
        _lib.call("lgs_mvp_transform_forward", _ptr(p), _ptr(vm), _ptr(pm), _ptr(_vl(valid_length)), V, N, _ptr(vp), _ptr(ndc), _stream(dev))
    return [vp, ndc]


def mvp_transform_backward(grad_ndc_pos, grad_view_pos, view_matrix, proj_matrix, view_pos, valid_length=None):
    gn = _f32c(grad_ndc_pos, "grad_ndc_pos"); gv = _f32c(grad_view_pos, "grad_view_pos")
    vm = _f32c(view_matrix, "view_matrix"); pm = _f32c(proj_matrix, "proj_matrix"); vp = _f32c(view_pos, "view_pos")
    V, N = gn.shape[0], gn.shape[2]
    dev = gn.device
    with torch.cuda.device(dev):
        out = torch.empty((4, N), dtype=_F32, device=dev)
        _lib.call("lgs_mvp_transform_backward", _ptr(gn), _ptr(gv), _ptr(vm), _ptr(pm), _ptr(vp), _ptr(_vl(valid_length)), V, N,
                  _ptr(out), _stream(dev))
    return out


def createTransformMatrix_forward(quaternion, scale, valid_length=None):
    q = _f32c(quaternion, "quaternion"); s = _f32c(scale, "scale")
    N = q.shape[1]
    dev = q.device
    with torch.cuda.device(dev):
        T = torch.empty((3, 3, N), dtype=_F32, device=dev)
        _lib.call("lgs_create_transform_matrix_forward", _ptr(q), _ptr(s), _ptr(_vl(valid_length)), N, _ptr(T), _stream(dev))
    return T


def createTransformMatrix_backward(transform_matrix_grad, quaternion, scale, valid_length=None):
    g = _f32c(transform_matrix_grad, "transform_matrix_grad"); q = _f32c(quaternion, "quaternion"); s = _f32c(scale, "scale")
    N = q.shape[1]
    dev = q.device
    with torch.cuda.device(dev):
        gq = torch.empty((4, N), dtype=_F32, device=dev)
        gs = torch.empty((3, N), dtype=_F32, device=dev)
        _lib.call("lgs_create_transform_matrix_backward", _ptr(g), _ptr(q), _ptr(s), _ptr(_vl(valid_length)), N, _ptr(gq), _ptr(gs),
                  _stream(dev))
    return [gq, gs]


def jacobianRayspace(translated_position, proj_matrix, output_h, output_w, valid_length=None):
    vp = _f32c(translated_position, "translated_position"); pm = _f32c(proj_matrix, "proj_matrix")
    V, N = vp.shape[0], vp.shape[2]
    dev = vp.device
    with torch.cuda.device(dev):
        J = torch.empty((V, 3, 3, N), dtype=_F32, device=dev)
        _lib.call("lgs_jacobian_rayspace", _ptr(vp), _ptr(pm), _ptr(_vl(valid_length)), V, N, int(output_h), int(output_w), _ptr(J),
                  _stream(dev))
    return J


def createCov2dDirectly_forward(J, view_matrix, transform_matrix, valid_length=None):
    j = _f32c(J, "J"); vm = _f32c(view_matrix, "view_matrix"); T = _f32c(transform_matrix, "transform_matrix")
    V, N = vm.shape[0], T.shape[2]
    dev = T.device
    with torch.cuda.device(dev):
        cov = torch.empty((V, 2, 2, N), dtype=_F32, device=dev)
        _lib.call("lgs_create_cov2d_forward", _ptr(j), _ptr(vm), _ptr(T), _ptr(_vl(valid_length)), V, N, _ptr(cov), _stream(dev))
    return cov


def createCov2dDirectly_backward(cov2d_grad, J, view_matrix, transform_matrix, valid_length=None):
    g = _f32c(cov2d_grad, "cov2d_grad"); j = _f32c(J, "J"); vm = _f32c(view_matrix, "view_matrix")
    T = _f32c(transform_matrix, "transform_matrix")
    V, N = vm.shape[0], T.shape[2]
    dev = T.device
    with torch.cuda.device(dev):
        gT = torch.empty((3, 3, N), dtype=_F32, device=dev)
        _lib.call("lgs_create_cov2d_backward", _ptr(g), _ptr(j), _ptr(vm), _ptr(T), _ptr(_vl(valid_length)), V, N, _ptr(gT), _stream(dev))
    return gT


def eigh_and_inv_2x2matrix_forward(input, valid_length=None):
    m = _f32c(input, "input")
    V, N = m.shape[0], m.shape[3]
    dev = m.device
    with torch.cuda.device(dev):
        val = torch.empty((V, 2, N), dtype=_F32, device=dev)
        vec = torch.empty((V, 2, 2, N), dtype=_F32, device=dev)
        inv = torch.empty((V, 2, 2, N), dtype=_F32, device=dev)
        _lib.call("lgs_eigh_and_inv_2x2_forward", _ptr(m), _ptr(_vl(valid_length)), V, N, _ptr(val), _ptr(vec), _ptr(inv), _stream(dev))
    return [val, vec, inv]


def inv_2x2matrix_backward(inv_matrix, dL_dInvMatrix, valid_length=None):
    a = _f32c(inv_matrix, "inv_matrix"); g = _f32c(dL_dInvMatrix, "dL_dInvMatrix")
    V, N = a.shape[0], a.shape[3]
    dev = a.device
    with torch.cuda.device(dev):
        out = torch.empty_like(g)
        _lib.call("lgs_inv_2x2_backward", _ptr(a), _ptr(g), _ptr(_vl(valid_length)), V, N, _ptr(out), _stream(dev))
    return out


def sh2rgb_forward(degree, sh_base, sh_rest, dir):
    s0 = _f32c(sh_base, "sh_base"); sr = _f32c(sh_rest, "sh_rest"); d = _f32c(dir, "dir")
    V, N = d.shape[0], d.shape[2]
    dev = d.device
    with torch.cuda.device(dev):
        rgb = torch.empty((V, 3, N), dtype=_F32, device=dev)
        _lib.call("lgs_sh2rgb_forward", int(degree), _ptr(s0), _ptr(sr), _ptr(d), V, N, _ptr(rgb), _stream(dev))
    return rgb


def sh2rgb_backward(degree, rgb_grad, sh_rest_dim, dir, SH_base, SH_rest):
    g = _f32c(rgb_grad, "rgb_grad"); d = _f32c(dir, "dir")
    V, N = g.shape[0], g.shape[2]
    dev = g.device
    with torch.cuda.device(dev):
        g0 = torch.empty((1, 3, N), dtype=_F32, device=dev)
        gr = torch.empty((int(sh_rest_dim), 3, N), dtype=_F32, device=dev)
        gd = torch.empty_like(d)
        _lib.call("lgs_sh2rgb_backward", int(degree), _ptr(g), int(sh_rest_dim), _ptr(d), V, N, _ptr(g0), _ptr(gr), _ptr(gd), _stream(dev))
    return [g0, gr, gd]



def get_allocate_size(ndc, view_space_z, inv_cov2d, opacity, height, width, tilesize_h, tilesize_w, valid_length=None):
    n = _f32c(ndc, "ndc"); z = _f32c(view_space_z, "view_space_z"); c = _f32c(inv_cov2d, "inv_cov2d"); o = _f32c(opacity, "opacity")
    V, N = n.shape[0], n.shape[2]
    dev = n.device
    with torch.cuda.device(dev):
        lu = torch.empty((V, 2, N), dtype=_I32, device=dev)
        rd = torch.empty((V, 2, N), dtype=_I32, device=dev)
        al = torch.empty((V, N), dtype=_I32, device=dev)
        _lib.call("lgs_get_allocate_size", _ptr(n), _ptr(z), _ptr(c), _ptr(o), _ptr(_vl(valid_length)), V, N, int(height), int(width),
                  int(tilesize_h), int(tilesize_w), _ptr(lu), _ptr(rd), _ptr(al), _stream(dev))
    return [lu, rd, al]


def create_table(ndc, inv_cov2d, opacity, offset, depth_sorted_pointid, feedback_buffer_cpu, idx_tensor_cpu,
                 height, width, tile_size_h, tile_size_w):
    n = _f32c(ndc, "ndc"); c = _f32c(inv_cov2d, "inv_cov2d"); o = _f32c(opacity, "opacity")
    off = _asc(offset, _I32, "offset"); sid = _asc(depth_sorted_pointid, _I64, "depth_sorted_pointid")
    V, N = n.shape[0], n.shape[2]
    dev = n.device
    with torch.cuda.device(dev):
        pred = 0
        if feedback_buffer_cpu is not None and idx_tensor_cpu is not None:
            for i in range(V):
                idx = int(idx_tensor_cpu[i])
                pred = max(pred, int(feedback_buffer_cpu[idx]))
                feedback_buffer_cpu[idx:idx + 1].copy_(off[i, N - 1:N], non_blocking=True)
        pred = int(1.5 * pred)
        if pred <= 0:
            pred = int(off[:, N - 1].max().item()) if N > 0 else 0
        if pred <= 0:
            raise RuntimeError("error pred_allocate_size")
        nbytes = ctypes.c_size_t(0)
        _lib.call("lgs_create_table_workspace_bytes", V, pred, ctypes.byref(nbytes))
        ws = torch.empty(nbytes.value, dtype=torch.uint8, device=dev)
        keys = torch.empty((V, pred), dtype=_I32, device=dev)
        vals = torch.empty((V, pred), dtype=_I32, device=dev)
        _lib.call("lgs_create_table", _ptr(n), _ptr(c), _ptr(o), _ptr(off), _ptr(sid), V, N, pred, int(height), int(width),
                  int(tile_size_h), int(tile_size_w), _ptr(keys), _ptr(vals), _ptr(ws), ctypes.c_size_t(nbytes.value), _stream(dev))
    return [keys, vals]


def tileRange(table_tileId, max_tileId):
    k = _asc(table_tileId, _I32, "table_tileId")
    V, L = k.shape
    dev = k.device
    with torch.cuda.device(dev):
        out = torch.empty((V, int(max_tileId) + 2), dtype=_I32, device=dev)
        _lib.call("lgs_tile_range", _ptr(k), V, L, int(max_tileId), int(CONFIG["fix_last_tile"]), _ptr(out), _stream(dev))
    return out



def _raster_forward_impl(sorted_points, start_index, packed, specific_tiles, img_h, img_w, th, tw,
                         enable_statistic, enable_trans, enable_depth):
    sp = _asc(sorted_points, _I32, "sorted_points"); si = _asc(start_index, _I32, "start_index")
    V, N = packed.shape[0], packed.shape[1]
    cap = sp.shape[1]
    gx, gy = _tiles(img_h, img_w, th, tw)
    Hp, Wp = gy * th, gx * tw
    if si.shape[1] != gx * gy + 2:
        raise RuntimeError(f"start_index has {si.shape[1]} entries, expected tiles+2 = {gx * gy + 2}")
    dev = packed.device
    tiles = None if specific_tiles is None else _asc(specific_tiles, _I32, "specific_tiles")
    n_sel = 0 if tiles is None else tiles.shape[1]
    img = torch.empty((V, 3, Hp, Wp), dtype=_F32, device=dev)
    T = torch.empty((V, 1, Hp, Wp), dtype=_F32, device=dev)
    if tiles is not None:
        img.zero_(); T.fill_(1.0)
    last = torch.zeros((V, 1, Hp, Wp), dtype=torch.int16, device=dev) if tiles is not None else \
        torch.empty((V, 1, Hp, Wp), dtype=torch.int16, device=dev)
    depth = torch.zeros((V, 1, Hp, Wp), dtype=_F32, device=dev) if enable_depth else torch.empty((0, 0, 0, 0), dtype=_F32, device=dev)
    fc = torch.zeros((V, 1, N), dtype=_I32, device=dev)
    fw = torch.zeros((V, 1, N), dtype=_F32, device=dev)
    _lib.call("lgs_rasterize_forward_packed", _ptr(sp), _ptr(si), _ptr(packed), _ptr(tiles), n_sel, V, N, cap, int(img_h), int(img_w),
              int(th), int(tw), int(bool(enable_statistic)), 0, _ptr(img), _ptr(T), _ptr(last), _ptr(fc), _ptr(fw), None, _stream(dev))
    return img, T, depth, last, fc, fw


def rasterize_forward(sorted_points, start_index, ndc, cov2d_inv, color, opacity, specific_tiles,
                      img_h, img_w, tilesize_h, tilesize_w, enable_statistic, enable_trans, enable_depth):
    n = _f32c(ndc, "ndc"); c = _f32c(cov2d_inv, "cov2d_inv"); col = _f32c(color, "color"); o = _f32c(opacity, "opacity")
    V, N = n.shape[0], n.shape[2]
    dev = n.device
    th, tw = int(tilesize_h), int(tilesize_w)
    with torch.cuda.device(dev):
        packed = torch.empty((V, N, 12), dtype=_F32, device=dev)
        _lib.call("lgs_pack_params", _ptr(n), _ptr(c), _ptr(col), _ptr(o), V, N, int(img_h), int(img_w), _ptr(packed), _stream(dev))
        img, T, depth, last, fc, fw = _raster_forward_impl(sorted_points, start_index, packed, specific_tiles, img_h, img_w, th, tw,
                                                           enable_statistic, enable_trans, enable_depth)
    return [img, T, depth, last, packed, fc, fw]


def rasterize_forward_packed(sorted_points, start_index, packed_params, specific_tiles, img_h, img_w, tile_h, tile_w,
                             enable_statistic, enable_trans, enable_depth):
    packed = _f32c(packed_params, "packed_params")
    if packed.shape[-1] != 12:
        raise RuntimeError("packed_params must be the f32[V,N,12] record produced by rasterize_forward")
    with torch.cuda.device(packed.device):
        img, T, depth, last, fc, fw = _raster_forward_impl(sorted_points, start_index, packed, specific_tiles, img_h, img_w,
                                                           int(tile_h), int(tile_w), enable_statistic, enable_trans, enable_depth)
    return [img, T, depth, last, fc, fw]


def rasterize_backward(sorted_points, start_index, packed_params, specific_tiles, final_transmitance, last_contributor,
                       d_img, d_trans_img_arg, d_depth_img_arg, grad_inv_sacler_arg,
                       img_h, img_w, tilesize_h, tilesize_w, enable_statistic):
    sp = _asc(sorted_points, _I32, "sorted_points"); si = _asc(start_index, _I32, "start_index")
    packed = _f32c(packed_params, "packed_params")
    T = _f32c(final_transmitance, "final_transmitance"); last = _asc(last_contributor, torch.int16, "last_contributor")
    g = _f32c(d_img, "d_img")
    gt = None if d_trans_img_arg is None else _f32c(d_trans_img_arg, "d_trans_img")
    sc = None if grad_inv_sacler_arg is None else _f32c(grad_inv_sacler_arg.reshape(1), "grad_inv_scaler")
    tiles = None if specific_tiles is None else _asc(specific_tiles, _I32, "specific_tiles")
    V, N = packed.shape[0], packed.shape[1]
    cap = sp.shape[1]
    dev = packed.device
    with torch.cuda.device(dev):
        pg = torch.empty((V, N, 12), dtype=_F32, device=dev)
        d_ndc = torch.empty((V, 4, N), dtype=_F32, device=dev)
        d_cov = torch.empty((V, 2, 2, N), dtype=_F32, device=dev)
        d_col = torch.empty((V, 3, N), dtype=_F32, device=dev)
        d_op = torch.empty((1, N), dtype=_F32, device=dev)
        e1 = torch.empty((V, 1, N), dtype=_F32, device=dev)
        e2 = torch.empty((V, 1, N), dtype=_F32, device=dev)
        _lib.call("lgs_rasterize_backward", _ptr(sp), _ptr(si), _ptr(packed), _ptr(tiles), 0 if tiles is None else tiles.shape[1],
                  _ptr(T), _ptr(last), _ptr(g), _ptr(gt), None, _ptr(sc), V, N, cap, int(img_h), int(img_w), int(tilesize_h),
                  int(tilesize_w), int(bool(enable_statistic)), _ptr(pg), _ptr(d_ndc), _ptr(d_cov), _ptr(d_col), _ptr(d_op),
                  _ptr(e1), _ptr(e2), _stream(dev))
    return [d_ndc, d_cov, d_col, d_op, e1, e2]



def adamUpdate(param, param_grad, exp_avg, exp_avg_sq, visible_index, valid_length, lr, b1, b2, eps):
    for name, t in (("param", param), ("exp_avg", exp_avg), ("exp_avg_sq", exp_avg_sq)):
        if not (t.is_cuda and t.dtype == _F32 and t.is_contiguous()):
            raise RuntimeError(f"adamUpdate: {name} must be a contiguous float32 CUDA tensor (updated in place)")
    g = _f32c(param_grad, "param_grad"); vi = _asc(visible_index, _I64, "visible_index")
    dev = param.device
    with torch.cuda.device(dev):
        if param.dim() == 3:
            R, C, S = param.shape
            A = vi.shape[0]
            _lib.call("lgs_adam_update_chunk", _ptr(param), _ptr(g), _ptr(exp_avg), _ptr(exp_avg_sq), _ptr(vi), _ptr(_vl(valid_length)),
                      R, C, S, A, float(lr), float(b1), float(b2), float(eps), _stream(dev))
        elif param.dim() == 2:
            R, N = param.shape
            _lib.call("lgs_adam_update_primitive", _ptr(param), _ptr(g), _ptr(exp_avg), _ptr(exp_avg_sq), _ptr(vi), R, N,
                      float(lr), float(b1), float(b2), float(eps), _stream(dev))
        else:
            raise RuntimeError("adamUpdate: param must be [R,chunks,chunk_size] or [R,N]")


def gpu_driven_pipeline_sparse_op(A, B, visible_chunk_ids, visible_count, op_name):
    for name, t in (("A", A), ("B", B), ("visible_chunk_ids", visible_chunk_ids), ("visible_count", visible_count)):
        if not t.is_cuda:
            raise RuntimeError(f"{name} must be a CUDA tensor")
    ops = {"add": 0, "sum": 0, "min": 1, "max": 2}
    if op_name not in ops:
        raise RuntimeError(f"Unsupported op: {op_name}. Expected: add, min, max")
    codes = {_F32: 0, _I32: 1, torch.float64: 2, _I64: 3, torch.int16: 4, torch.int8: 5, torch.uint8: 6}
    if A.dtype != B.dtype or A.dtype not in codes:
        raise RuntimeError(f"gpu_driven_pipeline_sparse_op: dtype {A.dtype}/{B.dtype} unsupported (expected one of {list(codes)})")
    if not A.is_contiguous():
        raise RuntimeError("gpu_driven_pipeline_sparse_op: A must be contiguous (updated in place)")
    Bc = B if B.is_contiguous() else B.contiguous()
    ids = _asc(visible_chunk_ids, _I64, "visible_chunk_ids"); cnt = _asc(visible_count, _I32, "visible_count")
    E, C, S = A.shape
    if S > 1024:
        raise RuntimeError("chunk_size exceeds max threads per block")
    dev = A.device
    with torch.cuda.device(dev):
        _lib.call("lgs_sparse_chunk_op", _ptr(A), _ptr(Bc), _ptr(ids), _ptr(cnt), codes[A.dtype], ops[op_name], E, C,
                  Bc.shape[1], S, _stream(dev))



def create_viewproj_forward(view_params, recp_tan_half_fov_x, img_h, img_w, z_near, z_far):
    vp = _f32c(view_params, "view_params"); rf = _f32c(recp_tan_half_fov_x.reshape(-1), "recp_tan_half_fov_x")
    if vp.dim() != 2 or vp.shape[1] != 7:
        raise RuntimeError(f"view_params must be [V,7], got {tuple(vp.shape)}")
    V = vp.shape[0]
    dev = vp.device
    with torch.cuda.device(dev):
        view = torch.empty((V, 4, 4), dtype=_F32, device=dev)
        proj = torch.empty((V, 4, 4), dtype=_F32, device=dev)
        viewproj = torch.empty((V, 4, 4), dtype=_F32, device=dev)
        planes = torch.empty((V, 6, 4), dtype=_F32, device=dev)
        _lib.call("lgs_create_viewproj_forward", _ptr(vp), _ptr(rf), V, int(img_h), int(img_w), float(z_near), float(z_far),
                  _ptr(view), _ptr(proj), _ptr(viewproj), _ptr(planes), _stream(dev))
    return [view, proj, viewproj, planes]


def create_viewproj_backward(view_matrix_grad, proj_matrix_grad, viewproj_matrix_grad, view_params, recp_tan_half_fov_x,
                             img_h, img_w, z_near, z_far):
    vp = _f32c(view_params, "view_params"); rf = _f32c(recp_tan_half_fov_x.reshape(-1), "recp_tan_half_fov_x")
    V = vp.shape[0]
    gv = _f32c(view_matrix_grad, "view_matrix_grad"); gp = _f32c(proj_matrix_grad, "proj_matrix_grad")
    gvp = _f32c(viewproj_matrix_grad, "viewproj_matrix_grad")
    for name, g in (("view_matrix_grad", gv), ("proj_matrix_grad", gp), ("viewproj_matrix_grad", gvp)):
        if g.numel() != V * 16:
            raise RuntimeError(f"{name} must be [V,4,4] with V = {V}, got {tuple(g.shape)}")
    dev = vp.device
    with torch.cuda.device(dev):
        g_params = torch.empty((V, 7), dtype=_F32, device=dev)
        g_recp = torch.zeros_like(rf)
        _lib.call("lgs_create_viewproj_backward", _ptr(gv), _ptr(gp), _ptr(gvp), _ptr(vp), _ptr(rf), V, int(img_h), int(img_w),
                  float(z_near), float(z_far), _ptr(g_params), _ptr(g_recp), _stream(dev))
    return [g_params, g_recp.reshape(recp_tan_half_fov_x.shape)]



def _out_of_scope(name, why):
    def fn(*args, **kwargs):
        raise NotImplementedError(f"litegs_fused.{name} is outside the render hot path rebuilt by litegs_b200: {why}")
    fn.__name__ = name
    return fn


world2ndc_forward = _out_of_scope("world2ndc_forward", "only reachable through the unused World2NdcFunc (wrapper.py:287)")
world2ndc_backword = _out_of_scope("world2ndc_backword", "only reachable through the unused World2NdcFunc (wrapper.py:287)")

EXPORTS = [
    "create_viewproj_forward", "create_viewproj_backward", "create_table", "tileRange", "get_allocate_size",
    "rasterize_forward", "rasterize_forward_packed", "rasterize_backward", "jacobianRayspace",
    "createTransformMatrix_forward", "createTransformMatrix_backward", "world2ndc_forward", "world2ndc_backword",
    "mvp_transform_forward", "mvp_transform_backward", "createCov2dDirectly_forward", "createCov2dDirectly_backward",
    "sh2rgb_forward", "sh2rgb_backward", "eigh_and_inv_2x2matrix_forward", "inv_2x2matrix_backward",
    "cull_compact_activate", "activate_backward", "adamUpdate", "frustum_culling_aabb", "gpu_driven_pipeline_sparse_op",
]
```

### litegs_b200/pipeline.py

```python
from __future__ import annotations

import ctypes
import os
from dataclasses import dataclass
from typing import Optional

import torch

from . import _lib
from .fused import CONFIG, _on, _ptr, _stream

_F32, _I32, _I64, _U8 = torch.float32, torch.int32, torch.int64, torch.uint8

_ws_bytes_cache: dict = {}
LAST_VIEW_SIZES: list = []


def _query_bytes(fn: str, *args) -> int:
    key = (fn,) + args
    v = _ws_bytes_cache.get(key)
    if v is None:
        n = ctypes.c_size_t(0)
        _lib.call(fn, *args, ctypes.byref(n))
        v = _ws_bytes_cache[key] = int(n.value)
    return v


def _round_up(n: int, m: int) -> int:
    return ((n + m - 1) // m) * m


@dataclass
class ViewState:
    sh_degree: int
    hw: tuple
    tile: tuple
    n_chunks_visible: int
    n_pairs: int
    chunk_ids: torch.Tensor
    counters: torch.Tensor
    view: torch.Tensor
    proj: torch.Tensor
    packed: torch.Tensor
    tile_count: torch.Tensor
    sorted_pid: torch.Tensor
    ranges: torch.Tensor
    T: torch.Tensor
    last: torch.Tensor
    tile_order: Optional[torch.Tensor] = None
    antialiased: bool = False
    filter_3d: Optional[torch.Tensor] = None


class _Pinned:
    _bufs: dict = {}

    @classmethod
    def get(cls, dev) -> torch.Tensor:
        b = cls._bufs.get(dev)
        if b is None:
            b = cls._bufs[dev] = torch.zeros(4, dtype=_I32).pin_memory()
        return b


def check_filter_3d(filter_3d: Optional[torch.Tensor], xyz: torch.Tensor) -> Optional[torch.Tensor]:
    if filter_3d is None:
        return None
    C, S = xyz.shape[-2:]
    if not (filter_3d.device == xyz.device and filter_3d.dtype == _F32 and filter_3d.is_contiguous()
            and tuple(filter_3d.shape[-2:]) == (C, S) and filter_3d.numel() == C * S):
        raise RuntimeError(f"filter_3d must be a contiguous float32 tensor of shape [1,{C},{S}] on {xyz.device}")
    return filter_3d.detach()


def render_view_forward(params: dict, cluster_origin: torch.Tensor, cluster_extend: torch.Tensor, frustumplane: torch.Tensor,
                        view_matrix: torch.Tensor, proj_matrix: torch.Tensor, sh_degree: int, hw: tuple, tile: tuple,
                        enable_statistic: bool = False, specific_tiles: Optional[torch.Tensor] = None, clamp_zero: bool = False,
                        antialiased: bool = False, filter_3d: Optional[torch.Tensor] = None):
    xyz = params["xyz"]
    dev = xyz.device
    filter_3d = check_filter_3d(filter_3d, xyz)
    C, S = xyz.shape[-2:]
    H, W = int(hw[0]), int(hw[1])
    th, tw = int(tile[0]), int(tile[1])
    if view_matrix.shape[0] != 1:
        raise RuntimeError("the fused pipeline renders one view per call (loop over views on the host)")
    for k in ("xyz", "scale", "rot", "sh_0", "sh_rest", "opacity"):
        t = params[k]
        if not (t.is_cuda and t.dtype == _F32 and t.is_contiguous()):
            raise RuntimeError(f"params['{k}'] must be a contiguous float32 CUDA tensor")
    gx, gy = (W + tw - 1) // tw, (H + th - 1) // th
    ntile = gx * gy
    Hp, Wp = gy * th, gx * tw
    M = C
    with _on(dev):
        st = _stream(dev)
        counters = torch.empty(4, dtype=_I32, device=dev)
        vis = torch.empty(M, dtype=_U8, device=dev)
        ids = torch.empty(M, dtype=_I64, device=dev)
        _lib.call("lgs_frustum_culling_aabb", _ptr(cluster_origin), _ptr(cluster_extend), _ptr(frustumplane), M, 1, _ptr(vis),
                  ctypes.c_void_p(counters.data_ptr()), _ptr(ids), st)
        Nmax = M * S
        packed = torch.empty((1, Nmax, 12), dtype=_F32, device=dev)
        dkey = torch.empty(Nmax, dtype=_I32, device=dev)
        iota = torch.empty(Nmax, dtype=_I32, device=dev)
        tcount = torch.empty(Nmax, dtype=_I32, device=dev)
        _lib.call("lgs_project_forward", int(sh_degree), _ptr(ids), ctypes.c_void_p(counters.data_ptr()), _ptr(view_matrix),
                  _ptr(proj_matrix), _ptr(xyz), _ptr(params["scale"]), _ptr(params["rot"]), _ptr(params["sh_0"]),
                  _ptr(params["sh_rest"]), _ptr(params["opacity"]), C, S, M, H, W, th, tw, _ptr(packed), _ptr(dkey), _ptr(iota),
                  _ptr(tcount), ctypes.c_void_p(counters.data_ptr() + 4), _ptr(filter_3d), int(bool(antialiased)), st)
        pinned = _Pinned.get(dev)
        pinned.copy_(counters, non_blocking=True)
        torch.cuda.current_stream(dev).synchronize()
        nvis, D = int(pinned[0]), int(pinned[1])
        kmin, kmax = ~int(pinned[2]) & 0xFFFFFFFF, int(pinned[3]) & 0xFFFFFFFF
        Nv = nvis * S
        LAST_VIEW_SIZES.append((D, max(1, (kmax - kmin).bit_length()) if (D > 0 and kmax >= kmin) else 1))
        if len(LAST_VIEW_SIZES) > 4096:
            del LAST_VIEW_SIZES[:2048]

        ranges = torch.empty((1, ntile + 2), dtype=_I32, device=dev)
        if D > 0:
            depth_bits = max(1, (kmax - kmin).bit_length()) if kmax >= kmin else 1
            nb = _query_bytes("lgs_sort_pairs_u32_workspace_bytes", _round_up(Nv, 1 << 16))
            ws = torch.empty(nb, dtype=_U8, device=dev)
            dkey_s = torch.empty(Nv, dtype=_I32, device=dev)
            order = torch.empty(Nv, dtype=_I32, device=dev)
            _lib.call("lgs_sort_pairs_u32_rebased", _ptr(dkey), _ptr(dkey_s), _ptr(iota), _ptr(order), Nv, kmin, depth_bits, _ptr(ws),
                      ctypes.c_size_t(nb), st)
            nb2 = _query_bytes("lgs_scan_gathered_workspace_bytes", _round_up(Nv, 1 << 16))
            ws2 = ws if nb2 <= nb else torch.empty(nb2, dtype=_U8, device=dev)
            offsets = dkey_s
            _lib.call("lgs_scan_gathered", _ptr(tcount), _ptr(order), Nv, _ptr(offsets), _ptr(ws2), ctypes.c_size_t(max(nb, nb2)), st)
            bits = ntile.bit_length()
            u16 = (ntile + 1) < 65536
            kdt = torch.int16 if u16 else _I32
            sfx = "_u16" if u16 else "_u32"
            keys = torch.empty(D, dtype=kdt, device=dev)
            vals = torch.empty(D, dtype=_I32, device=dev)
            _lib.call("lgs_emit_pairs_u16" if u16 else "lgs_emit_pairs", _ptr(packed), _ptr(offsets), _ptr(order), Nv, D, H, W, th, tw,
                      _ptr(keys), _ptr(vals), st)
            nb3 = _query_bytes(f"lgs_sort_pairs{sfx}_workspace_bytes", _round_up(D, 1 << 18))
            ws3 = ws if nb3 <= nb else torch.empty(nb3, dtype=_U8, device=dev)
            keys_s = torch.empty((1, D), dtype=kdt, device=dev)
            sorted_pid = torch.empty((1, D), dtype=_I32, device=dev)
            _lib.call(f"lgs_sort_pairs{sfx}", _ptr(keys), _ptr(keys_s), _ptr(vals), _ptr(sorted_pid), D, 0, bits, _ptr(ws3),
                      ctypes.c_size_t(max(nb, nb3)), st)
            _lib.call("lgs_tile_range_u16" if u16 else "lgs_tile_range", _ptr(keys_s), 1, D, ntile, 1, _ptr(ranges), st)
        else:
            sorted_pid = torch.zeros((1, 1), dtype=_I32, device=dev)
            _lib.call("lgs_tile_range", None, 1, 0, ntile, 1, _ptr(ranges), st)

        img = torch.empty((1, 3, Hp, Wp), dtype=_F32, device=dev)
        T = torch.empty((1, 1, Hp, Wp), dtype=_F32, device=dev)
        last = torch.empty((1, 1, Hp, Wp), dtype=torch.int16, device=dev)
        n_sel = 0
        if specific_tiles is not None:
            n_sel = specific_tiles.shape[1]
            img.zero_(); T.fill_(1.0); last.zero_()
        stats = None
        fc = fw = None
        if enable_statistic:
            fc = torch.zeros((1, 1, Nmax), dtype=_I32, device=dev)
            fw = torch.zeros((1, 1, Nmax), dtype=_F32, device=dev)
            stats = (fc, fw)
        order = None
        work = torch.empty((1, ntile), dtype=_I32, device=dev) if (CONFIG["tile_order"] and specific_tiles is None and D > 0) else None
        _lib.call("lgs_rasterize_forward_packed", _ptr(sorted_pid), _ptr(ranges), _ptr(packed), _ptr(specific_tiles), n_sel, 1,
                  Nmax, sorted_pid.shape[1], H, W, th, tw, int(bool(enable_statistic)), int(bool(clamp_zero)), _ptr(img), _ptr(T),
                  _ptr(last), _ptr(fc), _ptr(fw), _ptr(work), st)
        if work is not None:
            order = torch.empty((1, ntile), dtype=_I32, device=dev)
            _lib.call("lgs_tile_order", _ptr(work), 1, ntile, _ptr(order), st)
    state = ViewState(sh_degree=int(sh_degree), hw=(H, W), tile=(th, tw), n_chunks_visible=nvis, n_pairs=D, chunk_ids=ids,
                      counters=counters, view=view_matrix, proj=proj_matrix, packed=packed, tile_count=tcount,
                      sorted_pid=sorted_pid, ranges=ranges, T=T, last=last, tile_order=order, antialiased=bool(antialiased),
                      filter_3d=filter_3d)
    return img, state, stats


def render_view_backward(params: dict, state: ViewState, d_img: torch.Tensor, d_trans: Optional[torch.Tensor] = None,
                         enable_statistic: bool = False, specific_tiles: Optional[torch.Tensor] = None,
                         accumulate_into: Optional[dict] = None, clamped_img: Optional[torch.Tensor] = None,
                         camera_grad: Optional[torch.Tensor] = None):
    xyz = params["xyz"]
    dev = xyz.device
    C, S = xyz.shape[-2:]
    H, W = state.hw
    th, tw = state.tile
    A = state.n_chunks_visible
    R = params["sh_rest"].shape[0]
    Nmax = state.packed.shape[1]
    if not (d_img.is_cuda and d_img.dtype == _F32):
        raise RuntimeError("d_img must be a float32 CUDA tensor")
    d_img = d_img if d_img.is_contiguous() else d_img.contiguous()
    if d_trans is not None:
        d_trans = d_trans if d_trans.is_contiguous() else d_trans.contiguous()
    if camera_grad is not None and not (camera_grad.is_cuda and camera_grad.dtype == _F32 and camera_grad.is_contiguous()
                                        and tuple(camera_grad.shape) == (2, 4, 4)):
        raise RuntimeError("camera_grad must be a contiguous float32 CUDA tensor of shape [2,4,4]")
    with _on(dev):
        st = _stream(dev)
        cam_partials = None if camera_grad is None else torch.empty((max(A, 1), 32), dtype=_F32, device=dev)
        cam_args = (_ptr(cam_partials), _ptr(camera_grad))
        pg = torch.empty((1, Nmax, 12), dtype=_F32, device=dev)
        if specific_tiles is None:
            specific_tiles = state.tile_order
        n_sel = 0 if specific_tiles is None else specific_tiles.shape[1]
        _lib.call("lgs_rasterize_backward", _ptr(state.sorted_pid), _ptr(state.ranges), _ptr(state.packed), _ptr(specific_tiles), n_sel,
                  _ptr(state.T), _ptr(state.last), _ptr(d_img), _ptr(d_trans), _ptr(clamped_img), None, 1, Nmax, state.sorted_pid.shape[1],
                  H, W, th, tw,
                  int(bool(enable_statistic)), _ptr(pg), None, None, None, None, None, None, st)
        if accumulate_into is not None:
            for k in ("xyz", "scale", "rot", "sh_0", "sh_rest", "opacity"):
                t = accumulate_into[k]
                if not (t.is_cuda and t.dtype == _F32 and t.is_contiguous() and tuple(t.shape) == tuple(params[k].shape)):
                    raise RuntimeError(f"accumulate_into['{k}'] must be a contiguous float32 CUDA tensor shaped like the parameter")
            if A > 0:
                d = accumulate_into
                _lib.call("lgs_project_backward", state.sh_degree, _ptr(state.chunk_ids), ctypes.c_void_p(state.counters.data_ptr()),
                          _ptr(state.view), _ptr(state.proj), _ptr(xyz), _ptr(params["scale"]), _ptr(params["rot"]),
                          _ptr(params["opacity"]), C, S, A, R, H, W, int(CONFIG["true_sigmoid_grad"]), _ptr(pg), None, 2,
                          _ptr(d["xyz"]), _ptr(d["scale"]), _ptr(d["rot"]), _ptr(d["sh_0"]), _ptr(d["sh_rest"]), _ptr(d["opacity"]),
                          _ptr(d.get("_touched")), *cam_args, _ptr(state.filter_3d), int(state.antialiased), st)
            elif camera_grad is not None:
                camera_grad.zero_()
            return None, pg
        g_pos = torch.empty((3, A, S), dtype=_F32, device=dev)
        g_sc = torch.empty((3, A, S), dtype=_F32, device=dev)
        g_rot = torch.empty((4, A, S), dtype=_F32, device=dev)
        g_s0 = torch.empty((1, 3, A, S), dtype=_F32, device=dev)
        K = (state.sh_degree + 1) ** 2
        g_sr = torch.zeros((R, 3, A, S), dtype=_F32, device=dev) if R > K - 1 else torch.empty((R, 3, A, S), dtype=_F32, device=dev)
        g_op = torch.empty((1, A, S), dtype=_F32, device=dev)
        if A > 0:
            _lib.call("lgs_project_backward", state.sh_degree, _ptr(state.chunk_ids), ctypes.c_void_p(state.counters.data_ptr()),
                      _ptr(state.view), _ptr(state.proj), _ptr(xyz), _ptr(params["scale"]), _ptr(params["rot"]), _ptr(params["opacity"]),
                      C, S, A, R, H, W, int(CONFIG["true_sigmoid_grad"]), _ptr(pg), None, 0, _ptr(g_pos), _ptr(g_sc), _ptr(g_rot),
                      _ptr(g_s0), _ptr(g_sr), _ptr(g_op), None, *cam_args, _ptr(state.filter_3d), int(state.antialiased), st)
        elif camera_grad is not None:
            camera_grad.zero_()
    return [g_pos, g_sc, g_rot, g_s0, g_sr, g_op], pg



GRAPHS_ENABLED = os.environ.get("LGS_GRAPHS", "1") != "0"
SYNC_FREE = os.environ.get("LGS_SYNC_FREE", "1") != "0"


class ViewWorkspace:

    def __init__(self, params: dict, hw: tuple, tile: tuple, pair_capacity: int, planned_depth_bits: int = 24, use_graphs: bool = True):
        xyz = params["xyz"]
        dev = xyz.device
        C, S = xyz.shape[-2:]
        H, W = int(hw[0]), int(hw[1])
        th, tw = int(tile[0]), int(tile[1])
        gx, gy = (W + tw - 1) // tw, (H + th - 1) // th
        self.dev, self.C, self.S, self.hw, self.tile = dev, C, S, (H, W), (th, tw)
        self.ntile, self.Hp, self.Wp = gx * gy, gy * th, gx * tw
        self.Nmax = C * S
        self.cap = int(max(1024, pair_capacity))
        self.planned_bits = int(planned_depth_bits)
        self.use_graphs = bool(use_graphs)
        self.u16 = (self.ntile + 1) < 65536
        kdt = torch.int16 if self.u16 else _I32
        N, D = self.Nmax, self.cap
        e = lambda shape, dt: torch.empty(shape, dtype=dt, device=dev)
        self.counters = torch.zeros(4, dtype=_I32, device=dev)
        self.vparams = torch.zeros(8, dtype=_I32, device=dev)
        self.vis, self.chunk_ids = e(C, _U8), e(C, _I64)
        self.packed, self.dkey, self.iota, self.tcount = e((1, N, 12), _F32), e(N, _I32), e(N, _I32), e(N, _I32)
        self.dkey_s, self.order = e(N, _I32), e(N, _I32)
        self.keys, self.vals, self.keys_s, self.sorted_pid = e(D, kdt), e(D, _I32), e((1, D), kdt), e((1, D), _I32)
        self.ranges = e((1, self.ntile + 2), _I32)
        self.img, self.T = e((1, 3, self.Hp, self.Wp), _F32), e((1, 1, self.Hp, self.Wp), _F32)
        self.last = e((1, 1, self.Hp, self.Wp), torch.int16)
        self.work, self.tile_order = e((1, self.ntile), _I32), e((1, self.ntile), _I32)
        self.pg = e((1, N, 12), _F32)
        self.d_img = e((1, 3, self.Hp, self.Wp), _F32)
        self.cam_view, self.cam_proj, self.cam_planes = e((1, 4, 4), _F32), e((1, 4, 4), _F32), e((1, 6, 4), _F32)
        self.cam_partials, self.d_cam = e((C, 32), _F32), e((2, 4, 4), _F32)
        nb = max(_query_bytes("lgs_sort_pairs_u32_workspace_bytes", _round_up(N, 1 << 16)),
                 _query_bytes("lgs_scan_gathered_workspace_bytes", _round_up(N, 1 << 16)),
                 _query_bytes(f"lgs_sort_pairs_{'u16' if self.u16 else 'u32'}_workspace_bytes", _round_up(D, 1 << 18)))
        self.ws, self.ws_bytes = e(nb, _U8), nb
        self.sticky = torch.zeros(4, dtype=_I32, device=dev)
        self.sticky_host = torch.zeros(4, dtype=_I32).pin_memory()
        self.sticky_event = None
        self._graphs = {}
        self._eager_runs = {}
        self.views_done = 0

    def _forward_kernels(self, params, cluster_origin, cluster_extend, sh_degree, clamp_zero, antialiased, filter_3d):
        dev, st = self.dev, _stream(self.dev)
        H, W = self.hw
        th, tw = self.tile
        C, S, N, D = self.C, self.S, self.Nmax, self.cap
        cnt = self.counters.data_ptr()
        vp = self.vparams.data_ptr()
        _lib.call("lgs_frustum_culling_aabb", _ptr(cluster_origin), _ptr(cluster_extend), _ptr(self.cam_planes), C, 1, _ptr(self.vis),
                  ctypes.c_void_p(cnt), _ptr(self.chunk_ids), st)
        _lib.call("lgs_project_forward", int(sh_degree), _ptr(self.chunk_ids), ctypes.c_void_p(cnt), _ptr(self.cam_view), _ptr(self.cam_proj),
                  _ptr(params["xyz"]), _ptr(params["scale"]), _ptr(params["rot"]), _ptr(params["sh_0"]), _ptr(params["sh_rest"]),
                  _ptr(params["opacity"]), C, S, C, H, W, th, tw, _ptr(self.packed), _ptr(self.dkey), _ptr(self.iota), _ptr(self.tcount),
                  ctypes.c_void_p(cnt + 4), _ptr(filter_3d), int(antialiased), st)
        _lib.call("lgs_view_params", ctypes.c_void_p(cnt), S, D, self.planned_bits, ctypes.c_void_p(vp), _ptr(self.sticky), st)
        n_dev, d_dev, bias_dev = ctypes.c_void_p(vp), ctypes.c_void_p(vp + 4), ctypes.c_void_p(vp + 8)
        wsz = ctypes.c_size_t(self.ws_bytes)
        _lib.call("lgs_sort_pairs_u32_dev", _ptr(self.dkey), _ptr(self.dkey_s), _ptr(self.iota), _ptr(self.order), N, n_dev, bias_dev,
                  self.planned_bits, _ptr(self.ws), wsz, st)
        offsets = self.dkey_s
        _lib.call("lgs_scan_gathered_dev", _ptr(self.tcount), _ptr(self.order), N, n_dev, _ptr(offsets), _ptr(self.ws), wsz, st)
        _lib.call("lgs_emit_pairs_dev", _ptr(self.packed), _ptr(offsets), _ptr(self.order), N, n_dev, D, H, W, th, tw, 16 if self.u16 else 32,
                  _ptr(self.keys), _ptr(self.vals), d_dev, st)
        bits = self.ntile.bit_length()
        _lib.call("lgs_sort_pairs_u16_dev" if self.u16 else "lgs_sort_pairs_u32k_dev", _ptr(self.keys), _ptr(self.keys_s), _ptr(self.vals),
                  _ptr(self.sorted_pid), D, d_dev, 0, bits, _ptr(self.ws), wsz, st)
        _lib.call("lgs_tile_range_u16_dev" if self.u16 else "lgs_tile_range_dev", _ptr(self.keys_s), D, d_dev, self.ntile,
                  int(CONFIG["fix_last_tile"]), _ptr(self.ranges), st)
        order = CONFIG["tile_order"]
        _lib.call("lgs_rasterize_forward_packed", _ptr(self.sorted_pid), _ptr(self.ranges), _ptr(self.packed), None, 0, 1, N, D, H, W, th, tw,
                  0, int(bool(clamp_zero)), _ptr(self.img), _ptr(self.T), _ptr(self.last), None, None, _ptr(self.work) if order else None, st)
        if order:
            _lib.call("lgs_tile_order", _ptr(self.work), 1, self.ntile, _ptr(self.tile_order), st)

    def _backward_kernels(self, params, sh_degree, accumulate_into, use_clamp, camera_grad, antialiased, filter_3d):
        st = _stream(self.dev)
        H, W = self.hw
        th, tw = self.tile
        C, S, N, D = self.C, self.S, self.Nmax, self.cap
        tiles = self.tile_order if CONFIG["tile_order"] else None
        _lib.call("lgs_rasterize_backward", _ptr(self.sorted_pid), _ptr(self.ranges), _ptr(self.packed), _ptr(tiles),
                  self.ntile if tiles is not None else 0, _ptr(self.T), _ptr(self.last), _ptr(self.d_img), None,
                  _ptr(self.img) if use_clamp else None, None, 1, N, D, H, W, th, tw, 0, _ptr(self.pg), None, None, None, None, None, None, st)
        d = accumulate_into
        R = params["sh_rest"].shape[0]
        _lib.call("lgs_project_backward", int(sh_degree), _ptr(self.chunk_ids), ctypes.c_void_p(self.counters.data_ptr()), _ptr(self.cam_view),
                  _ptr(self.cam_proj), _ptr(params["xyz"]), _ptr(params["scale"]), _ptr(params["rot"]), _ptr(params["opacity"]), C, S, C, R,
                  H, W, int(CONFIG["true_sigmoid_grad"]), _ptr(self.pg), None, 2, _ptr(d["xyz"]), _ptr(d["scale"]), _ptr(d["rot"]),
                  _ptr(d["sh_0"]), _ptr(d["sh_rest"]), _ptr(d["opacity"]), _ptr(d.get("_touched")),
                  _ptr(self.cam_partials) if camera_grad else None, _ptr(self.d_cam) if camera_grad else None, _ptr(filter_3d),
                  int(antialiased), st)

    def _run(self, kind, sig, fn):
        key = (kind, sig)
        graphs = self.use_graphs and GRAPHS_ENABLED
        g = self._graphs.get(key) if graphs else None
        if g is not None:
            g.replay()
            return
        seen = self._eager_runs.get(key, 0)
        cur = torch.cuda.current_stream(self.dev)
        if not graphs or seen < 1 or cur.cuda_stream == 0:
            self._eager_runs[key] = seen + 1
            fn()
            return
        g = torch.cuda.CUDAGraph()
        with torch.cuda.graph(g, stream=cur, capture_error_mode="thread_local"):
            fn()
        self._graphs[key] = g
        g.replay()

    def forward(self, params, cluster_origin, cluster_extend, cam, sh_degree, clamp_zero=True, antialiased=False, filter_3d=None):
        filter_3d = check_filter_3d(filter_3d, params["xyz"])
        self.cam_view.copy_(cam["view"], non_blocking=True)
        self.cam_proj.copy_(cam["proj"], non_blocking=True)
        self.cam_planes.copy_(cam["frustumplane"], non_blocking=True)
        sig = (tuple(params[k].data_ptr() for k in ("xyz", "scale", "rot", "sh_0", "sh_rest", "opacity")), cluster_origin.data_ptr(),
               cluster_extend.data_ptr(), int(sh_degree), bool(clamp_zero), bool(CONFIG["tile_order"]),
               0 if filter_3d is None else filter_3d.data_ptr(), bool(antialiased))
        self._run("fwd", sig, lambda: self._forward_kernels(params, cluster_origin, cluster_extend, sh_degree, clamp_zero, antialiased,
                                                            filter_3d))
        self.views_done += 1
        return self.img

    def backward(self, params, d_img, sh_degree, accumulate_into, use_clamp=True, camera_grad=None, antialiased=False, filter_3d=None):
        filter_3d = check_filter_3d(filter_3d, params["xyz"])
        if camera_grad is not None and not (camera_grad.is_cuda and camera_grad.dtype == _F32 and tuple(camera_grad.shape) == (2, 4, 4)):
            raise RuntimeError("camera_grad must be a float32 CUDA tensor of shape [2,4,4]")
        H, W = self.hw
        if d_img.shape[-2:] == (self.Hp, self.Wp):
            self.d_img.copy_(d_img, non_blocking=True)
        else:
            if self.Hp != H or self.Wp != W:
                self.d_img.zero_()
            self.d_img[..., :H, :W].copy_(d_img, non_blocking=True)
        sig = (tuple(params[k].data_ptr() for k in ("xyz", "scale", "rot", "sh_0", "sh_rest", "opacity")),
               tuple(accumulate_into[k].data_ptr() for k in ("xyz", "scale", "rot", "sh_0", "sh_rest", "opacity")),
               0 if accumulate_into.get("_touched") is None else accumulate_into["_touched"].data_ptr(), int(sh_degree), bool(use_clamp),
               bool(CONFIG["tile_order"]), bool(antialiased), 0 if filter_3d is None else filter_3d.data_ptr(), camera_grad is not None)
        cam = camera_grad is not None
        self._run("bwd", sig, lambda: self._backward_kernels(params, sh_degree, accumulate_into, use_clamp, cam, antialiased, filter_3d))
        if cam:
            camera_grad.copy_(self.d_cam, non_blocking=True)

    def post_flags(self):
        self.sticky_host.copy_(self.sticky, non_blocking=True)
        self.sticky.zero_()
        self.sticky_event = torch.cuda.Event()
        self.sticky_event.record(torch.cuda.current_stream(self.dev))

    def check(self, wait: bool = False):
        ev = self.sticky_event
        if ev is None:
            return None
        if not ev.query():
            if not wait:
                return None
            ev.synchronize()
        self.sticky_event = None
        flags, pairs, bits, views = (int(x) for x in self.sticky_host)
        if flags:
            raise CapacityExceeded(pairs=pairs, pair_capacity=self.cap, depth_bits=bits, planned_depth_bits=self.planned_bits)
        return {"max_pairs": pairs, "max_depth_bits": bits, "views": views}


class CapacityExceeded(RuntimeError):
    def __init__(self, pairs, pair_capacity, depth_bits, planned_depth_bits):
        super().__init__(f"view workspace too small: {pairs} (tile, splat) pairs for a capacity of {pair_capacity}, depth keys span {depth_bits} "
                         f"bits with {planned_depth_bits} planned; grow the workspace and redo the step")
        self.pairs, self.pair_capacity, self.depth_bits, self.planned_depth_bits = pairs, pair_capacity, depth_bits, planned_depth_bits


def probe_view_sizes(params, cluster_origin, cluster_extend, cams, sh_degree, hw, tile, antialiased=False, filter_3d=None):
    max_pairs, max_bits = 0, 1
    p = {k: params[k].detach() for k in ("xyz", "scale", "rot", "sh_0", "sh_rest", "opacity")}
    with torch.no_grad():
        for cam in cams:
            _, st, _ = render_view_forward(p, cluster_origin, cluster_extend, cam["frustumplane"], cam["view"], cam["proj"], sh_degree, hw, tile,
                                           antialiased=antialiased, filter_3d=filter_3d)
            max_pairs = max(max_pairs, st.n_pairs)
            c = st.counters.cpu()
            kmin, kmax = ~int(c[2]) & 0xFFFFFFFF, int(c[3]) & 0xFFFFFFFF
            if st.n_pairs > 0 and kmax >= kmin:
                max_bits = max(max_bits, max(1, (kmax - kmin).bit_length()))
    return max_pairs, max_bits
```

Before: 882.0.

## Record per-chunk contribution bitmask in forward raster and skip dead splats in backward

The forward rasterizer now keeps a per-warp bitmask of which splats in each 32-entry chunk actually contributed to any pixel and writes one word per chunk to a new mask buffer. The backward kernel reads this mask and only walks the marked splats, skipping the compute and atomics for splats that contributed nothing. The flush path is also reworked with precomputed shared-memory addresses and inline PTX loads, and tile_work becomes the count of marked splats so tile ordering follows the reduced backward work. This adds a mask write and extra bookkeeping to the forward pass and changes the kernel signatures.

```diff
diff --git a/include/litegs_b200.h b/include/litegs_b200.h
--- a/include/litegs_b200.h
+++ b/include/litegs_b200.h
@@ -125,7 +125,7 @@
                                  const int* specific_tiles, int n_specific, int V, int N, int cap, int img_h, int img_w,
                                  int tile_h, int tile_w, int enable_statistic, int clamp_zero, float* img,
                                  float* transmittance, short* last_contributor, int* fragment_count,
-                                 float* fragment_weight, int* tile_work, void* stream);
+                                 float* fragment_weight, int* tile_work, unsigned* contrib_mask, void* stream);
 
 int lgs_tile_order(const int* work, int V, int ntile, int* order, void* stream);
 
@@ -134,7 +134,8 @@
                            const short* last_contributor, const float* d_img, const float* d_trans_img,
                            const float* clamped_img, const float* grad_inv_scaler, int V, int N, int cap, int img_h, int img_w, int tile_h,
                            int tile_w, int enable_statistic, float* packed_grad, float* d_ndc, float* d_cov2d_inv,
-                           float* d_color, float* d_opacity, float* err_sum, float* err_square_sum, void* stream);
+                           float* d_color, float* d_opacity, float* err_sum, float* err_square_sum, const unsigned* contrib_mask,
+                           void* stream);
 
 int lgs_set_staging(int bulk);
 int lgs_set_backward_reduce(int deferred);
diff --git a/litegs_b200/_lib.py b/litegs_b200/_lib.py
--- a/litegs_b200/_lib.py
+++ b/litegs_b200/_lib.py
@@ -46,10 +46,10 @@
     "lgs_tile_range_u16_dev": [_P, _I, _P, _I, _I, _P, _P],
     "lgs_tile_range_dev": [_P, _I, _P, _I, _I, _P, _P],
     "lgs_pack_params": [_P, _P, _P, _P, _I, _I, _I, _I, _P, _P],
-    "lgs_rasterize_forward_packed": [_P, _P, _P, _P, _I, _I, _I, _I, _I, _I, _I, _I, _I, _I, _P, _P, _P, _P, _P, _P, _P],
+    "lgs_rasterize_forward_packed": [_P, _P, _P, _P, _I, _I, _I, _I, _I, _I, _I, _I, _I, _I, _P, _P, _P, _P, _P, _P, _P, _P],
     "lgs_tile_order": [_P, _I, _I, _P, _P],
     "lgs_rasterize_backward": [_P, _P, _P, _P, _I, _P, _P, _P, _P, _P, _P, _I, _I, _I, _I, _I, _I, _I, _I,
-                               _P, _P, _P, _P, _P, _P, _P, _P],
+                               _P, _P, _P, _P, _P, _P, _P, _P, _P],
     "lgs_set_staging": [_I],
     "lgs_set_sort_impl": [_I],
     "lgs_set_radix_form": [_I],
diff --git a/litegs_b200/csrc/raster.cu b/litegs_b200/csrc/raster.cu
--- a/litegs_b200/csrc/raster.cu
+++ b/litegs_b200/csrc/raster.cu
@@ -25,25 +25,43 @@
 __device__ __forceinline__ float2 fma2(float2 a, float2 b, float2 c) { return make_float2(__fmaf_rn(a.x, b.x, c.x), __fmaf_rn(a.y, b.y, c.y)); }
 
 __device__ __forceinline__ void blend_pixel(float a, float cr, float cg, float cb, float& Ts, float& Cr, float& Cg, float& Cb,
-                                            float& nf, float ts_min, float a_min, float neg_ki)
+                                            float& nf, unsigned& hit, unsigned bit, float ts_min, float a_min, float neg_ki)
 {
     asm("{\n"
         ".reg .pred pa, pk;\n"
         ".reg .f32 w;\n"
-        "setp.gt.f32 pa, %0, %9;\n"
+        "setp.gt.f32 pa, %0, %10;\n"
         "@pa add.f32 %4, %4, 0f3F800000;\n"
-        "setp.ge.and.f32 pk, %5, %10, pa;\n"
-        "mul.f32 w, %5, %0;\n"
-        "@pk fma.rn.f32 %1, %6, w, %1;\n"
-        "@pk fma.rn.f32 %2, %7, w, %2;\n"
-        "@pk fma.rn.f32 %3, %8, w, %3;\n"
-        "@pk fma.rn.f32 %0, %11, w, %0;\n"
+        "setp.ge.and.f32 pk, %6, %11, pa;\n"
+        "mul.f32 w, %6, %0;\n"
+        "@pk fma.rn.f32 %1, %7, w, %1;\n"
+        "@pk fma.rn.f32 %2, %8, w, %2;\n"
+        "@pk fma.rn.f32 %3, %9, w, %3;\n"
+        "@pk fma.rn.f32 %0, %12, w, %0;\n"
+        "@pk or.b32 %5, %5, %13;\n"
         "}\n"
-        : "+f"(Ts), "+f"(Cr), "+f"(Cg), "+f"(Cb), "+f"(nf)
-        : "f"(a), "f"(cr), "f"(cg), "f"(cb), "f"(ts_min), "f"(a_min), "f"(neg_ki));
+        : "+f"(Ts), "+f"(Cr), "+f"(Cg), "+f"(Cb), "+f"(nf), "+r"(hit)
+        : "f"(a), "f"(cr), "f"(cg), "f"(cb), "f"(ts_min), "f"(a_min), "f"(neg_ki), "r"(bit));
 }
 
 __device__ __forceinline__ unsigned smem_u32(const void* p) { return (unsigned)__cvta_generic_to_shared(p); }
+template <int OFF> __device__ __forceinline__ void sts_f32(unsigned a, float v)
+{
+    asm volatile("st.shared.f32 [%0+%2], %1;\n" ::"r"(a), "f"(v), "n"(OFF) : "memory");
+}
+__device__ __forceinline__ void sts_s32(unsigned a, int v) { asm volatile("st.shared.s32 [%0], %1;\n" ::"r"(a), "r"(v) : "memory"); }
+template <int OFF> __device__ __forceinline__ float4 lds_f4(unsigned a)
+{
+    float4 v;
+    asm volatile("ld.shared.v4.f32 {%0, %1, %2, %3}, [%4+%5];\n" : "=f"(v.x), "=f"(v.y), "=f"(v.z), "=f"(v.w) : "r"(a), "n"(OFF) : "memory");
+    return v;
+}
+__device__ __forceinline__ int lds_s32(unsigned a)
+{
+    int v;
+    asm volatile("ld.shared.s32 %0, [%1];\n" : "=r"(v) : "r"(a) : "memory");
+    return v;
+}
 __device__ __forceinline__ void cp_async16(void* dst, const void* src)
 {
     asm volatile("cp.async.cg.shared.global [%0], [%1], 16;\n" ::"r"(smem_u32(dst)), "l"(src));
@@ -100,9 +118,9 @@
             __syncwarp();
         }
     }
-    __device__ __forceinline__ void issue(int which, const SplatRec* __restrict__ recs, int id)
+    __device__ __forceinline__ void issue(int which, const SplatRec* __restrict__ recs, int id, int slot)
     {
-        SplatRec* dst = buf + which * 32 + lane;
+        SplatRec* dst = buf + which * 32 + slot;
         if (BULK) {
             unsigned live = __ballot_sync(FULL_MASK, id >= 0);
             if (lane == 0) mbar_expect_tx(&bar[which], (unsigned)__popc(live) * (unsigned)sizeof(SplatRec));
@@ -120,22 +138,22 @@
         }
     }
     template <bool PRE = false>
-    __device__ __forceinline__ void wait(int which, bool more_in_flight)
+    __device__ __forceinline__ void wait(int which, bool more_in_flight, int slot = -1)
     {
         if (BULK) {
             mbar_wait(&bar[which], (phase_bits >> which) & 1u);
             phase_bits ^= (1u << which);
             pending &= ~(1u << which);
-            if (PRE) { prescale(which); __syncwarp(); }
+            if (PRE) { if (slot >= 0) prescale(which, slot); __syncwarp(); }
         } else {
             if (more_in_flight) cp_async_wait<1>(); else cp_async_wait<0>();
-            if (PRE) prescale(which);
+            if (PRE && slot >= 0) prescale(which, slot);
             __syncwarp();
         }
     }
-    __device__ __forceinline__ void prescale(int which)
+    __device__ __forceinline__ void prescale(int which, int slot)
     {
-        SplatRec* r = buf + which * 32 + lane;
+        SplatRec* r = buf + which * 32 + slot;
         const float2 ab = *reinterpret_cast<const float2*>(&r->A);
         const float2 co = *reinterpret_cast<const float2*>(&r->C);
         *reinterpret_cast<float2*>(&r->A) = make_float2((-0.5f * LOG2E) * ab.x, (-LOG2E) * ab.y);
@@ -170,12 +188,14 @@
     recs[(size_t)b * N + i] = r;
 }
 
+#define LGS_MASK_WORDS(cap, ntile) (((cap) >> 5) + (ntile) + 1)
+
 template <int TH, int TW, bool STAT, bool BULK, bool PAIRS = false>
-__global__ void __launch_bounds__(32 * WARPS_PER_BLOCK) raster_forward_kernel(
+__global__ void __launch_bounds__(32 * WARPS_PER_BLOCK, 1) raster_forward_kernel(
     const int* __restrict__ sorted, const int* __restrict__ start_index, const SplatRec* __restrict__ recs,
     const int* __restrict__ tiles, int n_sel, float* __restrict__ img, float* __restrict__ Tout, unsigned short* __restrict__ last,
-    int* __restrict__ frag_count, float* __restrict__ frag_weight, int* __restrict__ tile_work, int gx, int ntile, int cap, int N,
-    int Hp, int Wp, int clamp_zero)
+    int* __restrict__ frag_count, float* __restrict__ frag_weight, int* __restrict__ tile_work, unsigned* __restrict__ mask, int gx,
+    int ntile, int cap, int N, int Hp, int Wp, int clamp_zero)
 {
     constexpr int PPT = TH * TW / 32;
     __shared__ __align__(128) SplatRec s_rec[WARPS_PER_BLOCK][2][32];
@@ -203,28 +223,33 @@
     float Ts[PPT], Cr[PPT], Cg[PPT], Cb[PPT], nf[PPT];
 #pragma unroll
     for (int j = 0; j < PPT; j++) { Ts[j] = KI; Cr[j] = Cg[j] = Cb[j] = 0.0f; nf[j] = 0.0f; }
+    int nset = 0;
 
     if (count > 0) {
         Stager<BULK> st;
         st.init(&s_rec[warp][0][0], &s_bar[warp][0], lane);
         const int nchunks = (count + 31) >> 5;
         int id_cur = (lane < count) ? ids[lane] : -1;
-        st.issue(0, recs, id_cur);
+        st.issue(0, recs, id_cur, lane);
         int id_next = (32 + lane < count) ? ids[32 + lane] : -1;
+        const int mw = (start >> 5) + tile_id - 1;
         bool done = false;
         for (int c = 0; c < nchunks && !done; c++) {
             const bool more = (c + 1 < nchunks);
             if (more) {
-                st.issue((c + 1) & 1, recs, id_next);
+                st.issue((c + 1) & 1, recs, id_next, lane);
                 int nn = (c + 2) * 32 + lane;
                 id_next = (nn < count) ? ids[nn] : -1;
             }
-            st.template wait<true>(c & 1, more);
+            st.template wait<true>(c & 1, more, lane);
             const SplatRec* chunk = &s_rec[warp][c & 1][0];
             const int nk = min(32, count - c * 32);
             int my_id = 0;
             if (STAT) my_id = ids[c * 32 + min(lane, nk - 1)];
-            for (int k = 0; k < nk; k++) {
+            unsigned hit = 0;
+            unsigned bit = 1u;
+#pragma unroll 4
+            for (int k = 0; k < nk; k++, bit += bit) {
                 if ((k & 3) == 0) {
                     float tmax = Ts[0];
 #pragma unroll
@@ -254,7 +279,9 @@
                         const bool act0 = Ts[2 * p] > TS_MIN, act1 = Ts[2 * p + 1] > TS_MIN;
                         if (act0) nf[2 * p] += 1.0f;
                         if (act1) nf[2 * p + 1] += 1.0f;
-                        const float2 aw = make_float2((act0 && a0 >= A_MIN_S) ? a0 : 0.0f, (act1 && a1 >= A_MIN_S) ? a1 : 0.0f);
+                        const bool ok0 = act0 && a0 >= A_MIN_S, ok1 = act1 && a1 >= A_MIN_S;
+                        if (ok0 || ok1) hit |= bit;
+                        const float2 aw = make_float2(ok0 ? a0 : 0.0f, ok1 ? a1 : 0.0f);
                         const float2 w = mul2(aw, make_float2(Ts[2 * p], Ts[2 * p + 1]));
                         const float2 r2 = fma2(cr2, w, make_float2(Cr[2 * p], Cr[2 * p + 1]));
                         const float2 g2 = fma2(cg2, w, make_float2(Cg[2 * p], Cg[2 * p + 1]));
@@ -273,7 +300,7 @@
                         const bool ok = (Ts[j] > TS_MIN) && (a >= A_MIN_S);
                         if (ok) { fcount++; wsum += a * Ts[j]; }
                     }
-                    blend_pixel(a, q1.z, q1.w, cb, Ts[j], Cr[j], Cg[j], Cb[j], nf[j], TS_MIN, A_MIN_S, -KI);
+                    blend_pixel(a, q1.z, q1.w, cb, Ts[j], Cr[j], Cg[j], Cb[j], nf[j], hit, bit, TS_MIN, A_MIN_S, -KI);
                 }
                 }
                 if (STAT) {
@@ -287,6 +314,9 @@
                     }
                 }
             }
+            const unsigned word = __reduce_or_sync(FULL_MASK, hit);
+            nset += __popc(word);
+            if (mask != nullptr && lane == 0) mask[(size_t)b * LGS_MASK_WORDS(cap, ntile) + mw + c] = word;
             __syncwarp();
         }
         st.drain();
@@ -307,7 +337,7 @@
         float m = nf[0];
 #pragma unroll
         for (int j = 1; j < PPT; j++) m = fmaxf(m, nf[j]);
-        const int mi = __reduce_max_sync(FULL_MASK, (int)fminf(m, 65535.0f));
+        const int mi = (mask != nullptr) ? nset : __reduce_max_sync(FULL_MASK, (int)fminf(m, 65535.0f));
         if (lane == 0) tile_work[(size_t)b * ntile + tile_id - 1] = mi;
     }
 }
@@ -411,14 +441,14 @@
     const int nchunks = (kmax + 31) >> 5;
     int c0 = nchunks - 1;
     int id_cur = (c0 * 32 + lane < kmax) ? ids[c0 * 32 + lane] : -1;
-    st.issue(0, recs, id_cur);
+    st.issue(0, recs, id_cur, lane);
     int id_next = (c0 >= 1) ? ids[(c0 - 1) * 32 + lane] : -1;
     for (int v = 0; v < nchunks; v++) {
         const int c = nchunks - 1 - v;
         const bool more = (c >= 1);
         const int id_this = id_cur;
         if (more) {
-            st.issue((v + 1) & 1, recs, id_next);
+            st.issue((v + 1) & 1, recs, id_next, lane);
             id_cur = id_next;
             id_next = (c >= 2) ? ids[(c - 2) * 32 + lane] : -1;
         }
@@ -509,11 +539,12 @@
     const int* __restrict__ sorted, const int* __restrict__ start_index, const SplatRec* __restrict__ recs,
     const int* __restrict__ tiles, int n_sel, const float* __restrict__ Tfinal, const unsigned short* __restrict__ last,
     const float* __restrict__ d_img, const float* __restrict__ d_trans, const float* __restrict__ clamped_img,
-    float* __restrict__ grad, int gx, int ntile, int cap, int N, int Hp, int Wp, int err_mode)
+    float* __restrict__ grad, const unsigned* __restrict__ mask, int gx, int ntile, int cap, int N, int Hp, int Wp, int err_mode)
 {
     constexpr int PPT = TH * TW / 32, NP = PPT / 2;
     static_assert(PPT % 2 == 0, "pixels per lane must pair up");
     constexpr int NV = STAT ? 10 : 9;
+    constexpr int ROWB = LGS_ROWF * 4;
     constexpr float KS = 256.0f / 255.0f, A_MIN_S = ALPHA_MIN * KS;
     __shared__ __align__(128) SplatRec s_rec[WARPS_PER_BLOCK][2][32];
     __shared__ __align__(8) uint64_t s_bar[WARPS_PER_BLOCK][2];
@@ -561,60 +592,82 @@
     kmax = __reduce_max_sync(FULL_MASK, kmax);
     if (kmax <= 0) return;
 
+    const int sp = lane / NV, vslot = lane - sp * NV;
+    const unsigned park0 = smem_u32(&s_acc[warp][0][lane]);
+    const unsigned frow = smem_u32(&s_acc[warp][min(lane, LGS_RG * NV - 1)][0]);
+    const unsigned pid_lane = smem_u32(&s_pid[warp][sp]), pid0 = smem_u32(&s_pid[warp][0]);
+    float* const gdst = grad + (size_t)vslot * (DET ? 2 : 1);
     int pend = 0;
+    unsigned park = park0, pidp = pid0;
     auto flush = [&]() {
         __syncwarp();
+        const float4 x0 = lds_f4<0>(frow), x1 = lds_f4<16>(frow), x2 = lds_f4<32>(frow), x3 = lds_f4<48>(frow);
+        const float4 x4 = lds_f4<64>(frow), x5 = lds_f4<80>(frow), x6 = lds_f4<96>(frow), x7 = lds_f4<112>(frow);
+        float2 p0 = add2(make_float2(x0.x, x0.y), make_float2(x0.z, x0.w));
+        float2 p1 = add2(make_float2(x1.x, x1.y), make_float2(x1.z, x1.w));
+        float2 p2 = add2(make_float2(x2.x, x2.y), make_float2(x2.z, x2.w));
+        float2 p3 = add2(make_float2(x3.x, x3.y), make_float2(x3.z, x3.w));
+        float2 p4 = add2(make_float2(x4.x, x4.y), make_float2(x4.z, x4.w));
+        float2 p5 = add2(make_float2(x5.x, x5.y), make_float2(x5.z, x5.w));
+        float2 p6 = add2(make_float2(x6.x, x6.y), make_float2(x6.z, x6.w));
+        float2 p7 = add2(make_float2(x7.x, x7.y), make_float2(x7.z, x7.w));
+        p0 = add2(p0, p1); p2 = add2(p2, p3); p4 = add2(p4, p5); p6 = add2(p6, p7);
+        p0 = add2(p0, p2); p4 = add2(p4, p6);
+        p0 = add2(p0, p4);
+        const float sum = p0.x + p0.y;
+        const int pid = lds_s32(pid_lane);
         if (lane < pend * NV) {
-            const float4* r4 = reinterpret_cast<const float4*>(&s_acc[warp][lane][0]);
-            const float4 x0 = r4[0], x1 = r4[1], x2 = r4[2], x3 = r4[3], x4 = r4[4], x5 = r4[5], x6 = r4[6], x7 = r4[7];
-            float2 p0 = add2(make_float2(x0.x, x0.y), make_float2(x0.z, x0.w));
-            float2 p1 = add2(make_float2(x1.x, x1.y), make_float2(x1.z, x1.w));
-            float2 p2 = add2(make_float2(x2.x, x2.y), make_float2(x2.z, x2.w));
-            float2 p3 = add2(make_float2(x3.x, x3.y), make_float2(x3.z, x3.w));
-            float2 p4 = add2(make_float2(x4.x, x4.y), make_float2(x4.z, x4.w));
-            float2 p5 = add2(make_float2(x5.x, x5.y), make_float2(x5.z, x5.w));
-            float2 p6 = add2(make_float2(x6.x, x6.y), make_float2(x6.z, x6.w));
-            float2 p7 = add2(make_float2(x7.x, x7.y), make_float2(x7.z, x7.w));
-            p0 = add2(p0, p1); p2 = add2(p2, p3); p4 = add2(p4, p5); p6 = add2(p6, p7);
-            p0 = add2(p0, p2); p4 = add2(p4, p6);
-            p0 = add2(p0, p4);
-            const float sum = p0.x + p0.y;
-            const int sp = lane / NV, v = lane - sp * NV;
-            const int pid = s_pid[warp][sp];
             if (DET) {
-                unsigned long long* gq = reinterpret_cast<unsigned long long*>(grad);
-                atomicAdd(&gq[(size_t)pid * LGS_GRAD_FLOATS + v], (unsigned long long)__double2ll_rn((double)sum * LGS_DET_SCALE));
+                unsigned long long* gq = reinterpret_cast<unsigned long long*>(gdst) + (size_t)pid * LGS_GRAD_FLOATS;
+                atomicAdd(gq, (unsigned long long)__double2ll_rn((double)sum * LGS_DET_SCALE));
             } else {
-                atomicAdd(&grad[(size_t)pid * LGS_GRAD_FLOATS + v], sum);
+                atomicAdd(gdst + (size_t)pid * LGS_GRAD_FLOATS, sum);
             }
         }
         __syncwarp();
         pend = 0;
+        park = park0;
+        pidp = pid0;
+    };
+    const unsigned* mw = (mask != nullptr) ? mask + (size_t)b * LGS_MASK_WORDS(cap, ntile) + (start >> 5) + tile_id - 1 : nullptr;
+    const unsigned lanes_below = (1u << lane) - 1u;
+    auto chunk_bits = [&](int c) -> unsigned {
+        const int nk = kmax - c * 32;
+        const unsigned lim = (nk >= 32) ? FULL_MASK : ((1u << nk) - 1u);
+        return (mw != nullptr) ? (mw[c] & lim) : lim;
     };
     Stager<false> st;
     st.init(&s_rec[warp][0][0], &s_bar[warp][0], lane);
     const int nchunks = (kmax + 31) >> 5;
     int c0 = nchunks - 1;
-    int id_cur = (c0 * 32 + lane < kmax) ? ids[c0 * 32 + lane] : -1;
-    st.issue(0, recs, id_cur);
+    unsigned m_cur = chunk_bits(c0);
+    int id_cur = ((m_cur >> lane) & 1u) ? ids[c0 * 32 + lane] : -1;
+    st.issue(0, recs, id_cur, __popc(m_cur & lanes_below));
     int id_next = (c0 >= 1) ? ids[(c0 - 1) * 32 + lane] : -1;
+    unsigned m_next = (c0 >= 1) ? chunk_bits(c0 - 1) : 0u;
     for (int v = 0; v < nchunks; v++) {
         const int c = nchunks - 1 - v;
         const bool more = (c >= 1);
         const int id_this = id_cur;
+        const unsigned m_this = m_cur;
         if (more) {
-            st.issue((v + 1) & 1, recs, id_next);
+            if (!((m_next >> lane) & 1u)) id_next = -1;
+            st.issue((v + 1) & 1, recs, id_next, __popc(m_next & lanes_below));
             id_cur = id_next;
+            m_cur = m_next;
             id_next = (c >= 2) ? ids[(c - 2) * 32 + lane] : -1;
-        }
-        st.template wait<true>(v & 1, more);
+            m_next = (c >= 2) ? chunk_bits(c - 2) : 0u;
+        }
+        st.template wait<true>(v & 1, more, id_this >= 0 ? __popc(m_this & lanes_below) : -1);
         const SplatRec* chunk = &s_rec[warp][v & 1][0];
-        const int nk = min(32, kmax - c * 32);
-        for (int kk = nk - 1; kk >= 0; kk--) {
+        unsigned rem = m_this;
+        for (int i = __popc(m_this) - 1; i >= 0; i--) {
+            const int kk = 31 - __clz(rem);
+            rem ^= 1u << kk;
             const int k = c * 32 + kk;
-            const float4 q0 = *reinterpret_cast<const float4*>(&chunk[kk].px);
-            const float4 q1 = *reinterpret_cast<const float4*>(&chunk[kk].C);
-            const float2 q2 = *reinterpret_cast<const float2*>(&chunk[kk].b);
+            const float4 q0 = *reinterpret_cast<const float4*>(&chunk[i].px);
+            const float4 q1 = *reinterpret_cast<const float4*>(&chunk[i].C);
+            const float2 q2 = *reinterpret_cast<const float2*>(&chunk[i].b);
             const float cb = q2.x;
             const float dx = q0.x - fx, dy0 = q0.y - fy0;
             const float a2 = q0.z, b2 = q0.w, c2 = q1.x;
@@ -673,18 +726,19 @@
             if (__any_sync(FULL_MASK, any)) {
                 const float m0 = s0.x + s0.y, m1 = s1.x + s1.y, m2 = s2.x + s2.y;
                 const float u0 = dx * m0;
-                if (lane == kk) s_pid[warp][pend] = id_this;
-                float* row = &s_acc[warp][pend * NV][lane];
-                row[0 * LGS_ROWF] = u0;
-                row[1 * LGS_ROWF] = m1;
-                row[2 * LGS_ROWF] = dx * u0;
-                row[3 * LGS_ROWF] = dx * m1;
-                row[4 * LGS_ROWF] = m2;
-                row[5 * LGS_ROWF] = dr.x + dr.y;
-                row[6 * LGS_ROWF] = dg.x + dg.y;
-                row[7 * LGS_ROWF] = db.x + db.y;
-                row[8 * LGS_ROWF] = m0;
-                if (STAT) row[9 * LGS_ROWF] = esq;
+                if (lane == kk) sts_s32(pidp, id_this);
+                sts_f32<0 * ROWB>(park, u0);
+                sts_f32<1 * ROWB>(park, m1);
+                sts_f32<2 * ROWB>(park, dx * u0);
+                sts_f32<3 * ROWB>(park, dx * m1);
+                sts_f32<4 * ROWB>(park, m2);
+                sts_f32<5 * ROWB>(park, dr.x + dr.y);
+                sts_f32<6 * ROWB>(park, dg.x + dg.y);
+                sts_f32<7 * ROWB>(park, db.x + db.y);
+                sts_f32<8 * ROWB>(park, m0);
+                if (STAT) sts_f32<9 * ROWB>(park, esq);
+                park += NV * ROWB;
+                pidp += 4;
                 pend++;
                 if (pend == LGS_RG) flush();
             }
@@ -861,7 +915,7 @@
                                             const int* specific_tiles, int n_specific, int V, int N, int cap, int img_h, int img_w,
                                             int tile_h, int tile_w, int enable_statistic, int clamp_zero, float* img,
                                             float* transmittance, short* last_contributor, int* fragment_count,
-                                            float* fragment_weight, int* tile_work, void* stream)
+                                            float* fragment_weight, int* tile_work, unsigned* contrib_mask, void* stream)
 {
     LGS_REQUIRE(lgs_tile_ok(tile_h, tile_w), "rasterize_forward: tile %dx%d not one of 8x16, 12x16, 16x16, 8x8", tile_h, tile_w);
     LGS_REQUIRE(V >= 1 && img_h > 0 && img_w > 0, "rasterize_forward: bad sizes V=%d H=%d W=%d", V, img_h, img_w);
@@ -875,9 +929,11 @@
     const SplatRec* recs = (const SplatRec*)packed_params;
     const bool bulk = use_bulk();
 #define FWD(S, B) raster_forward_kernel<TH, TW, S, B><<<grid, block, 0, st>>>(sorted_points, start_index, recs, specific_tiles, n_specific, \
-        img, transmittance, (unsigned short*)last_contributor, fragment_count, fragment_weight, tile_work, gx, ntile, cap, N, Hp, Wp, clamp_zero)
+        img, transmittance, (unsigned short*)last_contributor, fragment_count, fragment_weight, tile_work, contrib_mask, gx, ntile, cap, N, Hp, \
+        Wp, clamp_zero)
 #define FWDP() raster_forward_kernel<TH, TW, false, false, true><<<grid, block, 0, st>>>(sorted_points, start_index, recs, specific_tiles, \
-        n_specific, img, transmittance, (unsigned short*)last_contributor, fragment_count, fragment_weight, tile_work, gx, ntile, cap, N, Hp, Wp, clamp_zero)
+        n_specific, img, transmittance, (unsigned short*)last_contributor, fragment_count, fragment_weight, tile_work, contrib_mask, gx, ntile, \
+        cap, N, Hp, Wp, clamp_zero)
     LGS_DISPATCH_TILE(tile_h, tile_w,
         if (enable_statistic) { if (bulk) FWD(true, true); else FWD(true, false); }
         else { if (bulk) FWD(false, true); else if (forward_pairs()) FWDP(); else FWD(false, false); })
@@ -893,7 +949,8 @@
                                       const float* clamped_img, const float* grad_inv_scaler, int V, int N, int cap, int img_h,
                                       int img_w, int tile_h,
                                       int tile_w, int enable_statistic, float* packed_grad, float* d_ndc, float* d_cov2d_inv,
-                                      float* d_color, float* d_opacity, float* err_sum, float* err_square_sum, void* stream)
+                                      float* d_color, float* d_opacity, float* err_sum, float* err_square_sum,
+                                      const unsigned* contrib_mask, void* stream)
 {
     LGS_REQUIRE(lgs_tile_ok(tile_h, tile_w), "rasterize_backward: tile %dx%d not one of 8x16, 12x16, 16x16, 8x8", tile_h, tile_w);
     LGS_REQUIRE(V >= 1 && img_h > 0 && img_w > 0, "rasterize_backward: bad sizes V=%d H=%d W=%d", V, img_h, img_w);
@@ -917,7 +974,7 @@
             LGS_CUDA(cudaMallocAsync((void**)&q, nq * sizeof(long long), st));
             LGS_CUDA(cudaMemsetAsync(q, 0, nq * sizeof(long long), st));
 #define BWD_DET(S, T) raster_backward_v2_kernel<TH, TW, S, T, true><<<grid, block, 0, st>>>(sorted_points, start_index, recs, specific_tiles, \
-        n_specific, final_transmittance, lastu, d_img, d_trans_img, clamped_img, (float*)q, gx, ntile, cap, N, Hp, Wp, g_err_mode)
+        n_specific, final_transmittance, lastu, d_img, d_trans_img, clamped_img, (float*)q, contrib_mask, gx, ntile, cap, N, Hp, Wp, g_err_mode)
             LGS_DISPATCH_TILE(tile_h, tile_w,
                 if (enable_statistic) { if (trans) BWD_DET(true, true); else BWD_DET(true, false); }
                 else { if (trans) BWD_DET(false, true); else BWD_DET(false, false); })
@@ -928,7 +985,7 @@
             LGS_CUDA(cudaFreeAsync(q, st));
         } else if (backward_version() == 2 && !bulk) {
 #define BW2(S, T) raster_backward_v2_kernel<TH, TW, S, T><<<grid, block, 0, st>>>(sorted_points, start_index, recs, specific_tiles, n_specific, \
-        final_transmittance, lastu, d_img, d_trans_img, clamped_img, packed_grad, gx, ntile, cap, N, Hp, Wp, g_err_mode)
+        final_transmittance, lastu, d_img, d_trans_img, clamped_img, packed_grad, contrib_mask, gx, ntile, cap, N, Hp, Wp, g_err_mode)
             LGS_DISPATCH_TILE(tile_h, tile_w,
                 if (enable_statistic) { if (trans) BW2(true, true); else BW2(true, false); }
                 else { if (trans) BW2(false, true); else BW2(false, false); })
diff --git a/litegs_b200/fused.py b/litegs_b200/fused.py
--- a/litegs_b200/fused.py
+++ b/litegs_b200/fused.py
@@ -345,7 +345,7 @@
     fc = torch.zeros((V, 1, N), dtype=_I32, device=dev)
     fw = torch.zeros((V, 1, N), dtype=_F32, device=dev)
     _lib.call("lgs_rasterize_forward_packed", _ptr(sp), _ptr(si), _ptr(packed), _ptr(tiles), n_sel, V, N, cap, int(img_h), int(img_w),
-              int(th), int(tw), int(bool(enable_statistic)), 0, _ptr(img), _ptr(T), _ptr(last), _ptr(fc), _ptr(fw), None, _stream(dev))
+              int(th), int(tw), int(bool(enable_statistic)), 0, _ptr(img), _ptr(T), _ptr(last), _ptr(fc), _ptr(fw), None, None, _stream(dev))
     return img, T, depth, last, fc, fw
 
 
@@ -398,7 +398,7 @@
         _lib.call("lgs_rasterize_backward", _ptr(sp), _ptr(si), _ptr(packed), _ptr(tiles), 0 if tiles is None else tiles.shape[1],
                   _ptr(T), _ptr(last), _ptr(g), _ptr(gt), None, _ptr(sc), V, N, cap, int(img_h), int(img_w), int(tilesize_h),
                   int(tilesize_w), int(bool(enable_statistic)), _ptr(pg), _ptr(d_ndc), _ptr(d_cov), _ptr(d_col), _ptr(d_op),
-                  _ptr(e1), _ptr(e2), _stream(dev))
+                  _ptr(e1), _ptr(e2), None, _stream(dev))
     return [d_ndc, d_cov, d_col, d_op, e1, e2]
 
 
diff --git a/litegs_b200/pipeline.py b/litegs_b200/pipeline.py
--- a/litegs_b200/pipeline.py
+++ b/litegs_b200/pipeline.py
@@ -28,6 +28,10 @@
 
 def _round_up(n: int, m: int) -> int:
     return ((n + m - 1) // m) * m
+
+
+def contrib_mask_words(cap: int, ntile: int) -> int:
+    return cap // 32 + ntile + 1
 
 
 @dataclass
@@ -50,6 +54,7 @@
     tile_order: Optional[torch.Tensor] = None
     antialiased: bool = False
     filter_3d: Optional[torch.Tensor] = None
+    contrib_mask: Optional[torch.Tensor] = None
 
 
 class _Pinned:
@@ -166,16 +171,17 @@
             stats = (fc, fw)
         order = None
         work = torch.empty((1, ntile), dtype=_I32, device=dev) if (CONFIG["tile_order"] and specific_tiles is None and D > 0) else None
+        mask = torch.empty(contrib_mask_words(sorted_pid.shape[1], ntile), dtype=_I32, device=dev)
         _lib.call("lgs_rasterize_forward_packed", _ptr(sorted_pid), _ptr(ranges), _ptr(packed), _ptr(specific_tiles), n_sel, 1,
                   Nmax, sorted_pid.shape[1], H, W, th, tw, int(bool(enable_statistic)), int(bool(clamp_zero)), _ptr(img), _ptr(T),
-                  _ptr(last), _ptr(fc), _ptr(fw), _ptr(work), st)
+                  _ptr(last), _ptr(fc), _ptr(fw), _ptr(work), _ptr(mask), st)
         if work is not None:
             order = torch.empty((1, ntile), dtype=_I32, device=dev)
             _lib.call("lgs_tile_order", _ptr(work), 1, ntile, _ptr(order), st)
     state = ViewState(sh_degree=int(sh_degree), hw=(H, W), tile=(th, tw), n_chunks_visible=nvis, n_pairs=D, chunk_ids=ids,
                       counters=counters, view=view_matrix, proj=proj_matrix, packed=packed, tile_count=tcount,
                       sorted_pid=sorted_pid, ranges=ranges, T=T, last=last, tile_order=order, antialiased=bool(antialiased),
-                      filter_3d=filter_3d)
+                      filter_3d=filter_3d, contrib_mask=mask)
     return img, state, stats
 
 
@@ -210,7 +216,7 @@
         _lib.call("lgs_rasterize_backward", _ptr(state.sorted_pid), _ptr(state.ranges), _ptr(state.packed), _ptr(specific_tiles), n_sel,
                   _ptr(state.T), _ptr(state.last), _ptr(d_img), _ptr(d_trans), _ptr(clamped_img), None, 1, Nmax, state.sorted_pid.shape[1],
                   H, W, th, tw,
-                  int(bool(enable_statistic)), _ptr(pg), None, None, None, None, None, None, st)
+                  int(bool(enable_statistic)), _ptr(pg), None, None, None, None, None, None, _ptr(state.contrib_mask), st)
         if accumulate_into is not None:
             for k in ("xyz", "scale", "rot", "sh_0", "sh_rest", "opacity"):
                 t = accumulate_into[k]
@@ -277,6 +283,7 @@
         self.img, self.T = e((1, 3, self.Hp, self.Wp), _F32), e((1, 1, self.Hp, self.Wp), _F32)
         self.last = e((1, 1, self.Hp, self.Wp), torch.int16)
         self.work, self.tile_order = e((1, self.ntile), _I32), e((1, self.ntile), _I32)
+        self.contrib_mask = e(contrib_mask_words(D, self.ntile), _I32)
         self.pg = e((1, N, 12), _F32)
         self.d_img = e((1, 3, self.Hp, self.Wp), _F32)
         self.cam_view, self.cam_proj, self.cam_planes = e((1, 4, 4), _F32), e((1, 4, 4), _F32), e((1, 6, 4), _F32)
@@ -321,7 +328,8 @@
                   int(CONFIG["fix_last_tile"]), _ptr(self.ranges), st)
         order = CONFIG["tile_order"]
         _lib.call("lgs_rasterize_forward_packed", _ptr(self.sorted_pid), _ptr(self.ranges), _ptr(self.packed), None, 0, 1, N, D, H, W, th, tw,
-                  0, int(bool(clamp_zero)), _ptr(self.img), _ptr(self.T), _ptr(self.last), None, None, _ptr(self.work) if order else None, st)
+                  0, int(bool(clamp_zero)), _ptr(self.img), _ptr(self.T), _ptr(self.last), None, None, _ptr(self.work) if order else None,
+                  _ptr(self.contrib_mask), st)
         if order:
             _lib.call("lgs_tile_order", _ptr(self.work), 1, self.ntile, _ptr(self.tile_order), st)
 
@@ -333,7 +341,8 @@
         tiles = self.tile_order if CONFIG["tile_order"] else None
         _lib.call("lgs_rasterize_backward", _ptr(self.sorted_pid), _ptr(self.ranges), _ptr(self.packed), _ptr(tiles),
                   self.ntile if tiles is not None else 0, _ptr(self.T), _ptr(self.last), _ptr(self.d_img), None,
-                  _ptr(self.img) if use_clamp else None, None, 1, N, D, H, W, th, tw, 0, _ptr(self.pg), None, None, None, None, None, None, st)
+                  _ptr(self.img) if use_clamp else None, None, 1, N, D, H, W, th, tw, 0, _ptr(self.pg), None, None, None, None, None, None,
+                  _ptr(self.contrib_mask), st)
         d = accumulate_into
         R = params["sh_rest"].shape[0]
         _lib.call("lgs_project_backward", int(sh_degree), _ptr(self.chunk_ids), ctypes.c_void_p(self.counters.data_ptr()), _ptr(self.cam_view),
diff --git a/profiles/microbench/raster_mask_bench.py b/profiles/microbench/raster_mask_bench.py
--- /dev/null
+++ b/profiles/microbench/raster_mask_bench.py
@@ -0,0 +1,87 @@
+import os
+import subprocess
+import sys
+
+sys.path.insert(0, os.path.dirname(os.path.dirname(os.path.dirname(os.path.abspath(__file__)))))
+import torch
+
+from litegs_b200 import _lib, pipeline, scene
+from litegs_b200.fused import _ptr, _stream
+
+KEYS = ("xyz", "scale", "rot", "sh_0", "sh_rest", "opacity")
+
+
+def main(n_views=8, reps=20):
+    dev = torch.device("cuda:0")
+    try:
+        plim = subprocess.run(["nvidia-smi", "--query-gpu=power.limit", "--format=csv,noheader"], capture_output=True, text=True).stdout.strip()
+    except OSError:
+        plim = "unknown"
+    print(f"GPU: {torch.cuda.get_device_name(0)}, power limit {plim}")
+    H, W, (th, tw) = 1080, 1920, (8, 16)
+    p = scene.make_scene(1_000_000, sh_degree=3, seed=0, log_scale_range=(0.002, 0.02))
+    P = {k: torch.from_numpy(p[k]).to(dev) for k in KEYS}
+    A = [torch.from_numpy(p[k]).to(dev) for k in ("cluster_origin", "cluster_extend")]
+    cams = [{k: torch.from_numpy(x).to(dev) for k, x in scene.make_camera(v, 64, W, H).items()} for v in range(n_views)]
+    g = torch.Generator(device="cpu").manual_seed(0)
+    views = []
+    for cam in cams:
+        img, st, _ = pipeline.render_view_forward(P, A[0], A[1], cam["frustumplane"], cam["view"], cam["proj"], 3, (H, W), (th, tw),
+                                                  clamp_zero=True)
+        d = torch.randn(img.shape, generator=g).to(dev)
+        views.append((st, d))
+    Hp, Wp = views[0][0].T.shape[-2:]
+    ntile = (Hp // th) * (Wp // tw)
+    Nmax = views[0][0].packed.shape[1]
+    img = torch.empty((1, 3, Hp, Wp), device=dev)
+    T = torch.empty((1, 1, Hp, Wp), device=dev)
+    last = torch.empty((1, 1, Hp, Wp), dtype=torch.int16, device=dev)
+    work = torch.empty((1, ntile), dtype=torch.int32, device=dev)
+    order = torch.empty((1, ntile), dtype=torch.int32, device=dev)
+    pg = torch.empty((1, Nmax, 12), device=dev)
+    st_ = _stream(dev)
+
+    def forward(st, mask):
+        _lib.call("lgs_rasterize_forward_packed", _ptr(st.sorted_pid), _ptr(st.ranges), _ptr(st.packed), None, 0, 1, Nmax,
+                  st.sorted_pid.shape[1], H, W, th, tw, 0, 1, _ptr(img), _ptr(T), _ptr(last), None, None, _ptr(work), _ptr(mask), st_)
+        _lib.call("lgs_tile_order", _ptr(work), 1, ntile, _ptr(order), st_)
+
+    def backward(st, d, mask):
+        _lib.call("lgs_rasterize_backward", _ptr(st.sorted_pid), _ptr(st.ranges), _ptr(st.packed), _ptr(order), ntile, _ptr(T), _ptr(last),
+                  _ptr(d), None, _ptr(img), None, 1, Nmax, st.sorted_pid.shape[1], H, W, th, tw, 0, _ptr(pg), None, None, None, None, None,
+                  None, _ptr(mask), st_)
+
+    def one_arm(masked):
+        e = [torch.cuda.Event(enable_timing=True) for _ in range(4 * n_views)]
+        for i, (st, d) in enumerate(views):
+            mask = st.contrib_mask if masked else None
+            e[4 * i].record(); forward(st, mask); e[4 * i + 1].record()
+            e[4 * i + 2].record(); backward(st, d, mask); e[4 * i + 3].record()
+        torch.cuda.synchronize()
+        return (sum(e[4 * i].elapsed_time(e[4 * i + 1]) for i in range(n_views)) / n_views,
+                sum(e[4 * i + 2].elapsed_time(e[4 * i + 3]) for i in range(n_views)) / n_views)
+
+    for _ in range(3):
+        one_arm(False); one_arm(True)
+    tf, tb = {False: [], True: []}, {False: [], True: []}
+    for r in range(reps):
+        for masked in ((False, True) if r % 2 == 0 else (True, False)):
+            f, b = one_arm(masked)
+            tf[masked].append(f); tb[masked].append(b)
+    med = lambda v: sorted(v)[len(v) // 2]
+    for name, t in (("lgs_rasterize_forward_packed (+ tile order)", tf), ("lgs_rasterize_backward", tb)):
+        print(f"C2 per-view {name}, median of {reps} x {n_views} views: NULL {med(t[False]):.4f} ms, mask {med(t[True]):.4f} ms "
+              f"({100 * (med(t[True]) / med(t[False]) - 1):+.2f} %); spread NULL {min(t[False]):.4f}-{max(t[False]):.4f}, "
+              f"mask {min(t[True]):.4f}-{max(t[True]):.4f} ms")
+    steps = marked = 0
+    for st, _ in views:
+        forward(st, st.contrib_mask)
+        kmax = last.to(torch.int64).bitwise_and(0xFFFF).view(Hp // th, th, Wp // tw, tw)
+        steps += int(kmax.amax(dim=(1, 3)).sum())
+        marked += int(work.sum())
+    torch.cuda.synchronize()
+    print(f"C2 backward steps over {n_views} views: {steps} in the full walk, {marked} marked ({100 * (1 - marked / steps):.1f} % skipped)")
+
+
+if __name__ == "__main__":
+    main()
```

New measurement: 900.5 (median of 6 runs). 1.02x the previous value.
